# leijue222/Intra-and-Inter-Human-Relation-Network-for-MPEE

Hardware: AMD Instinct MI355X
Metric: images/sec (256x192 crops) I2R-Net HRNet-W48 inference (higher is better)
Workload: dtype f32; 1 GPU; vanilla I2R-Net HRNet-W48-S 256x192, 6 encoder layers, fp32, random weights (BASELINE configs[1]: w48_pure_en6); images_per_gpu=8, persons_per_image=4, crops_per_gpu_step=32, parallelism=single GPU, programs_per_forward=3

## Files before the change

intra-and-inter-human-relation-network-for-mpee_amd/csrc/i2r_conv.h:

```cpp
#pragma once
#include "i2r_common.h"

#ifdef I2R_TUNING
#define I2R_DBG(p) ((p).dbg)
#else
#define I2R_DBG(p) 0
#endif

namespace {

struct ConvK {
    const float* in;
    const float* in2;
    const float* w;
    const float* bias;
    const float* res1;
    const float* res2;
    const float* res_post;
    float* out;
    int n_img, in_h, in_w, in_cs, cin;
    int conv_h, conv_w, out_h, out_w, out_cs, cout, cout_pad;
    int stride, iy0, ix0, ntaps;
    int tap_kh, tap_kw;
    int out_step, out_off_y, out_off_x, rep, relu;
    int tile_h, tile_w, tiles_y, tiles_x, n_cblk;
    int ph, pw, plane;
    int ck;
    int wn;
    int dtype;
    int in16, out16;
    int dbg;
    unsigned m_cblk, m_tx, m_ty, m_pw, m_tw;
    unsigned in_bytes, w_bytes, out_bytes;
    int wn_log, npass;
    int algo, w_fwlog, w_pitch, w_half, w_nfrag, w_rcp;
    int w_seq;
    int w_band;
    unsigned w_m_cblk, w_m_img, w_m_tx;
    const float* f_t1;
    const float* f_t2;
    float* f_y;
    int f_sh1, f_sh2;
    unsigned f_bytes1, f_bytes2;
};

__device__ __forceinline__ int div_m(int n, int d, unsigned m) { return d == 1 ? n : (int)__umulhi((unsigned)n, m); }

typedef unsigned u32x4 __attribute__((ext_vector_type(4)));
typedef unsigned u32x2 __attribute__((ext_vector_type(2)));
constexpr unsigned kOOB = 0x80000000u;
__device__ __forceinline__ __amdgpu_buffer_rsrc_t make_rsrc(const void* base, unsigned bytes) {
    return __builtin_amdgcn_make_buffer_rsrc(const_cast<void*>(base), 0, base ? bytes : 0, 0x00020000);
}
__device__ __forceinline__ f32x4 buf_ld16(const __amdgpu_buffer_rsrc_t& rs, unsigned voff, int soff) {
    return __builtin_bit_cast(f32x4, __builtin_amdgcn_raw_buffer_load_b128(rs, voff, soff, 0));
}
__device__ __forceinline__ void buf_st16(const __amdgpu_buffer_rsrc_t& rs, unsigned voff, int soff, f32x4 v) {
    __builtin_amdgcn_raw_buffer_store_b128(__builtin_bit_cast(u32x4, v), rs, voff, soff, 0);
    asm volatile("s_nop 1" ::"v"(v));
}

constexpr int kMaxPP = 5;

constexpr int kMaxGroups = 4;
struct ConvGroupK {
    ConvK g[kMaxGroups];
    int blk_end[kMaxGroups];
    int n;
    const int* blk_map;
};

template <int DT>
__device__ __forceinline__ f32x4 ld_act4(const float* base, size_t off, bool h16) {
    if constexpr (DT != 0) {
        if (h16) {
            const uint2 u = *reinterpret_cast<const uint2*>(reinterpret_cast<const unsigned short*>(base) + off);
            if constexpr (DT == 1)
                return (f32x4){__uint_as_float(u.x << 16), __uint_as_float(u.x & 0xFFFF0000u), __uint_as_float(u.y << 16), __uint_as_float(u.y & 0xFFFF0000u)};
            else {
                typedef _Float16 h4 __attribute__((ext_vector_type(4)));
                const h4 h = __builtin_bit_cast(h4, u);
                return (f32x4){(float)h[0], (float)h[1], (float)h[2], (float)h[3]};
            }
        }
    }
    return *reinterpret_cast<const f32x4*>(base + off);
}
template <int DT>
__device__ __forceinline__ void st_act4(float* base, size_t off, f32x4 v, bool h16) {
    if constexpr (DT != 0) {
        if (h16) {
            uint2 u;
            if constexpr (DT == 1) {
                typedef __bf16 b4 __attribute__((ext_vector_type(4)));
                const b4 b = {(__bf16)v[0], (__bf16)v[1], (__bf16)v[2], (__bf16)v[3]};
                u = __builtin_bit_cast(uint2, b);
            } else {
                typedef _Float16 h4 __attribute__((ext_vector_type(4)));
                const h4 h = {(_Float16)v[0], (_Float16)v[1], (_Float16)v[2], (_Float16)v[3]};
                u = __builtin_bit_cast(uint2, h);
            }
            *reinterpret_cast<uint2*>(reinterpret_cast<unsigned short*>(base) + off) = u;
            return;
        }
    }
    *reinterpret_cast<f32x4*>(base + off) = v;
}

template <int DT>
__device__ __forceinline__ f32x4 buf_ld_act4(const __amdgpu_buffer_rsrc_t& rs, unsigned voff, bool h16) {
    if constexpr (DT != 0) {
        if (h16) {
            const u32x2 u = __builtin_amdgcn_raw_buffer_load_b64(rs, voff, 0, 0);
            if constexpr (DT == 1)
                return (f32x4){__uint_as_float(u.x << 16), __uint_as_float(u.x & 0xFFFF0000u), __uint_as_float(u.y << 16), __uint_as_float(u.y & 0xFFFF0000u)};
            else {
                typedef _Float16 h4 __attribute__((ext_vector_type(4)));
                const h4 h = __builtin_bit_cast(h4, u);
                return (f32x4){(float)h[0], (float)h[1], (float)h[2], (float)h[3]};
            }
        }
    }
    return buf_ld16(rs, voff, 0);
}
template <int DT>
__device__ __forceinline__ void buf_st_act4(const __amdgpu_buffer_rsrc_t& rs, unsigned voff, f32x4 v, bool h16) {
    if constexpr (DT != 0) {
        if (h16) {
            u32x2 u;
            if constexpr (DT == 1) {
                typedef __bf16 b4 __attribute__((ext_vector_type(4)));
                const b4 b = {(__bf16)v[0], (__bf16)v[1], (__bf16)v[2], (__bf16)v[3]};
                u = __builtin_bit_cast(u32x2, b);
            } else {
                typedef _Float16 h4 __attribute__((ext_vector_type(4)));
                const h4 h = {(_Float16)v[0], (_Float16)v[1], (_Float16)v[2], (_Float16)v[3]};
                u = __builtin_bit_cast(u32x2, h);
            }
            __builtin_amdgcn_raw_buffer_store_b64(u, rs, voff, 0, 0);
            return;
        }
    }
    __builtin_amdgcn_raw_buffer_store_b128(__builtin_bit_cast(u32x4, v), rs, voff, 0, 0);
}

template <int MT, int NT, int DT>
__device__ __forceinline__ void conv_epilogue(const ConvK& p, f32x4 (&acc)[MT][NT], int img, int oy0, int ox0, int wm, int n_base,
                                              int li, int g, int tile_px) {
    if ((I2R_DBG(p) & 1) && acc[0][0][0] != 12345.678f) return;
    const int j4 = li & 3;
    const int pj = li >> 2, pq = li & 3;
    const int perm_src = (g * 16 + pq * 4 + pj) * 4;
    auto to_pixel_major = [&](f32x4 v) {
        v = quad_transpose(v, j4);
#pragma unroll
        for (int e = 0; e < 4; ++e) {
            const float x = v[e];
            v[e] = __int_as_float(__builtin_amdgcn_ds_bpermute(perm_src, __float_as_int(x)));
        }
        return v;
    };
    const bool h16 = DT != 0 && p.out16;
    const unsigned esz = h16 ? 2u : 4u;
    const __amdgpu_buffer_rsrc_t rs_out = make_rsrc(p.out, p.out_bytes), rs_r1 = make_rsrc(p.res1, p.out_bytes),
                                 rs_r2 = make_rsrc(p.res2, p.out_bytes), rs_rp = make_rsrc(p.res_post, p.out_bytes);
    auto finish = [&](f32x4 t, int n, bool full, unsigned voff) {
        if (p.relu == 1) {
            t[0] = fmaxf(t[0], 0.f); t[1] = fmaxf(t[1], 0.f); t[2] = fmaxf(t[2], 0.f); t[3] = fmaxf(t[3], 0.f);
        } else if (p.relu == 2) {
#pragma unroll
            for (int e = 0; e < 4; ++e) t[e] = 0.5f * t[e] * (1.f + erff(t[e] * 0.70710678118654752f));
        }
        if (p.res_post) t += buf_ld_act4<DT>(rs_rp, voff, h16);
        if (!full) {
#pragma unroll
            for (int e = 0; e < 4; ++e)
                if (n + e >= p.cout) t[e] = 0.f;
        }
        return t;
    };
    f32x4 bias[NT];
    unsigned noff[NT];
    const bool tail = n_base + NT * 16 > p.cout || n_base + NT * 16 > p.out_cs;
#pragma unroll
    for (int nt = 0; nt < NT; ++nt) {
        const int n = n_base + nt * 16 + pq * 4;
        const bool nok = n < p.cout_pad && (n + 4 <= p.cout || n + 4 <= p.out_cs);
        noff[nt] = nok ? (unsigned)n * esz : kOOB;
        bias[nt] = n < p.cout_pad ? *reinterpret_cast<const f32x4*>(p.bias + n) : (f32x4){0.f, 0.f, 0.f, 0.f};
    }
    if (p.rep == 1 && !(I2R_DBG(p) & 16)) {
        unsigned off[MT];
#pragma unroll
        for (int mt = 0; mt < MT; ++mt) {
            const int m = (wm * MT + mt) * 16 + g * 4 + pj;
            const int ty = div_m(m, p.tile_w, p.m_tw), tx = m - ty * p.tile_w;
            const int oy = oy0 + ty, ox = ox0 + tx;
            const bool pv = m < tile_px && oy < p.conv_h && ox < p.conv_w;
            off[mt] = pv ? (unsigned)(((img * p.out_h + oy * p.out_step + p.out_off_y) * p.out_w + ox * p.out_step + p.out_off_x) * p.out_cs) * esz : kOOB;
        }
        auto at = [&](int mt, int nt) { return (tail && noff[nt] == kOOB) ? kOOB : off[mt] + noff[nt]; };
        f32x4 r[MT][NT];
#pragma unroll
        for (int mt = 0; mt < MT; ++mt)
#pragma unroll
            for (int nt = 0; nt < NT; ++nt) {
                r[mt][nt] = bias[nt];
                if (p.res1) r[mt][nt] += buf_ld_act4<DT>(rs_r1, at(mt, nt), h16);
                if (p.res2) r[mt][nt] += buf_ld_act4<DT>(rs_r2, at(mt, nt), h16);
            }
#pragma unroll
        for (int mt = 0; mt < MT; ++mt)
#pragma unroll
            for (int nt = 0; nt < NT; ++nt) {
// ... 42 lines not shown
```

intra-and-inter-human-relation-network-for-mpee_amd/csrc/i2r_conv.hip:

```cpp
#include <stdlib.h>

#include <algorithm>

#include "i2r_conv.h"

namespace {

template <int MT, int NT, int CAP, int PF>
__device__ __forceinline__ void conv_body(const ConvK& p, int bid, f32x4* lds) {
    const int tid = threadIdx.x;
    unsigned long long ts0 = 0, ts1 = 0, ts2 = 0;
    const bool stamp = (I2R_DBG(p) & 8) != 0;
    const int bid_stamp = bid;
    if (stamp) ts0 = __builtin_amdgcn_s_memtime();
    const int lane = tid & 63, wave = tid >> 6;
    const int WN = p.wn;
    const int wm = wave >> p.wn_log, wn = wave & (WN - 1);
    const int li = lane & 15, g = lane >> 4;

    int q = div_m(bid, p.n_cblk, p.m_cblk);
    const int cb = bid - q * p.n_cblk;
    bid = q;
    q = div_m(bid, p.tiles_x, p.m_tx);
    const int tile_x = bid - q * p.tiles_x;
// ... 134 lines not shown
        }
    } else {
        for (int c0 = 0; c0 < p.cin; c0 += p.ck) {
            const int ckc = min(p.ck, p.cin - c0);
            const int ncg = ckc >> 2;
            if (c0 != 0) __syncthreads();
            for (int cg0 = 0; cg0 < ncg; cg0 += 4) {
                f32x4 v[4][kMaxPP];
#pragma unroll
                for (int u = 0; u < 4; ++u)
#pragma unroll
                    for (int j = 0; j < kMaxPP; ++j)
                        v[u][j] = (j < npp && !(I2R_DBG(p) & 2)) ? buf_ld16(rs_in, goff[j] + u * 16u, (c0 + cg0 * 4) * 4) : (f32x4){0.f, 0.f, 0.f, 0.f};
                if (p.in2) {
#pragma unroll
                    for (int u = 0; u < 4; ++u)
#pragma unroll
                        for (int j = 0; j < kMaxPP; ++j)
                            if (j < npp) v[u][j] += buf_ld16(rs_in2, goff[j] + u * 16u, (c0 + cg0 * 4) * 4);
                }
#pragma unroll
                for (int u = 0; u < 4; ++u)
#pragma unroll
                    for (int j = 0; j < kMaxPP; ++j) {
                        const int pp = tid + j * 256;
                        if (j < npp && pp < phw)
                            lds[(cg0 + u) * p.plane + pp] = v[u][j];
                    }
            }
            __syncthreads();
            run_chunk(lds, c0, ckc, []() {});
        }
    }

    if (stamp) {
        ts2 = __builtin_amdgcn_s_memtime();
        ConvK q = p;
        q.res2 = nullptr;
        conv_epilogue<MT, NT, 0>(q, acc, img, oy0, ox0, wm, n_base, li, g, tile_px);
        asm volatile("s_waitcnt vmcnt(0)" ::: "memory");
        const unsigned long long ts3 = __builtin_amdgcn_s_memtime();
        if (tid == 0) {
            unsigned long long* o = reinterpret_cast<unsigned long long*>(const_cast<float*>(p.res2)) + (size_t)bid_stamp * 4;
            o[0] = ts0; o[1] = ts1; o[2] = ts2; o[3] = ts3;
            if (I2R_DBG(p) & 32) {
                const unsigned hw = __builtin_amdgcn_s_getreg((4 << 0) | (0 << 6) | (31 << 11));
                const unsigned xcc = __builtin_amdgcn_s_getreg((20 << 0) | (0 << 6) | (3 << 11));
                o[1] = ((unsigned long long)xcc << 32) | hw;
            }
        }
        return;
    }
    conv_epilogue<MT, NT, 0>(p, acc, img, oy0, ox0, wm, n_base, li, g, tile_px);
}

template <int MT, int NT, int CAP, int PF>
__global__ __launch_bounds__(256) void conv_igemm_f32(const ConvGroupK grp) {
    extern __shared__ __attribute__((aligned(16))) f32x4 lds[];
    int bid = blockIdx.x, gi = 0, start = 0;
    if (grp.blk_map) {
        const int v = __builtin_amdgcn_readfirstlane(grp.blk_map[bid]);
        gi = v >> 24;
        bid = v & 0xFFFFFF;
    } else {
#pragma unroll
        for (int i = 0; i < kMaxGroups - 1; ++i)
            if (i + 1 < grp.n && bid >= grp.blk_end[i]) { gi = i + 1; start = grp.blk_end[i]; }
    }
    conv_body<MT, NT, CAP, PF>(grp.g[gi], bid - start, lds);
}

template <int NT, int CAP, int PF>
conv_fn pick_mt(int mt) {
    switch (mt) {
        case 1: return conv_igemm_f32<1, NT, CAP, PF>;
        case 2: return conv_igemm_f32<2, NT, CAP, PF>;
        case 3: return conv_igemm_f32<3, NT, CAP, PF>;
        case 4: return conv_igemm_f32<4, NT, CAP, PF>;
    }
    return nullptr;
}

template <int CAP, int PF>
conv_fn pick_nt(int nt, int mt) {
    switch (nt) {
        case 3: return pick_mt<3, CAP, PF>(mt);
        case 4: return pick_mt<4, CAP, PF>(mt);
        case 5: return pick_mt<5, CAP, PF>(mt);
    }
    return nullptr;
}

conv_fn pick_kernel(int nt, int mt, int cap, int pf) {
    if (pf == 0) return pick_nt<4, 0>(nt, mt);
    if (pf == 1 && cap == 4) return pick_nt<4, 1>(nt, mt);
    if (pf == 1 && cap == 12) return pick_nt<12, 1>(nt, mt);
    if (pf == 2 && cap == 4) return pick_nt<4, 2>(nt, mt);
    return nullptr;
}

inline int cdiv(int a, int b) { return (a + b - 1) / b; }

}

static void copy_desc(const i2r_conv_desc* d, ConvK& k) {
    k.in = d->in; k.in2 = d->in2; k.w = d->w; k.bias = d->bias; k.res1 = d->res1; k.res2 = d->res2; k.res_post = d->res_post; k.out = d->out;
    k.n_img = d->n_img; k.in_h = d->in_h; k.in_w = d->in_w; k.in_cs = d->in_cs; k.cin = d->cin;
    k.conv_h = d->conv_h; k.conv_w = d->conv_w; k.out_h = d->out_h; k.out_w = d->out_w; k.out_cs = d->out_cs;
    k.cout = d->cout; k.cout_pad = d->cout_pad; k.stride = d->stride; k.iy0 = d->iy0; k.ix0 = d->ix0;
    k.ntaps = d->ntaps;
    k.out_step = d->out_step; k.out_off_y = d->out_off_y; k.out_off_x = d->out_off_x; k.rep = d->rep; k.relu = d->relu;
    k.dtype = d->dtype;
    k.in16 = d->in_f16; k.out16 = d->out_f16;
    k.algo = d->algo; k.w_fwlog = k.w_pitch = k.w_half = k.w_nfrag = k.w_rcp = k.w_band = 0; k.w_seq = 1;
    k.w_m_cblk = k.w_m_img = k.w_m_tx = 0; k.in_bytes = k.w_bytes = k.out_bytes = 0;
    k.m_cblk = k.m_tx = k.m_ty = k.m_pw = k.m_tw = 0; k.wn_log = 0; k.npass = 0;
    k.dbg = 0;
    k.f_t1 = d->t1; k.f_t2 = d->t2; k.f_y = d->y; k.f_sh1 = d->t1_shift; k.f_sh2 = d->t2 ? d->t2_shift : 0; k.f_bytes1 = k.f_bytes2 = 0;
}

constexpr int kWinoMaxSeq = 8;
constexpr int kWinoRunPasses = 6;
constexpr int kWinoMinWg = 512;
static long long wino_runs(const ConvK& k, int mt) { return (((long long)k.w_nfrag + mt - 1) / mt + k.w_seq - 1) / k.w_seq; }

static int prepare_wino(const i2r_conv_desc* d, int force_mt, ConvK& k, int* nt_out, int* mt_out, int* cap_out, int* pf_out, size_t* lds_out,
                        long long* nblk_out) {
    I2R_CHECK_ARG(d->dtype == 0 && !d->in_f16 && !d->out_f16, "i2r_conv: the Winograd kernels are fp32");
    I2R_CHECK_ARG(d->stride == 1 && d->ntaps == 9 && d->iy0 == -1 && d->ix0 == -1 && d->rep == 1 && d->out_step == 1 && d->out_off_y == 0 &&
                      d->out_off_x == 0 && d->in2 == nullptr,
                  "i2r_conv: algo 1 (Winograd) needs a plain 3x3 stride-1 pad-1 convolution");
    for (int t = 0; t < 9; ++t) I2R_CHECK_ARG(d->dy[t] == t / 3 && d->dx[t] == t % 3, "i2r_conv: algo 1 needs row-major 3x3 taps");
    I2R_CHECK_ARG(d->relu == 0 || d->relu == 1, "i2r_conv: algo 1 has no GELU epilogue");
    I2R_CHECK_ARG((long long)d->n_img * d->in_h * d->in_w * d->in_cs < (1ll << 29) && (long long)d->n_img * d->out_h * d->out_w * d->out_cs < (1ll << 29) &&
                      (long long)16 * d->cin * d->cout_pad < (1ll << 29),
                  "i2r_conv: algo 1 addresses its tensors through buffer descriptors of < 2 GiB");
    I2R_CHECK_ARG(d->conv_h == d->in_h && d->conv_w == d->in_w && d->out_h == d->conv_h && d->out_w == d->conv_w, "i2r_conv: algo 1 geometry");
    if (d->t1) {
        I2R_CHECK_ARG(d->y != nullptr, "i2r_conv: a fused input (t1) needs y");
        I2R_CHECK_ARG(d->in_cs == d->cin, "i2r_conv: fused input: y is complete only when the conv reads every channel (cin=%d in_cs=%d)", d->cin, d->in_cs);
        for (int t = 0; t < (d->t2 ? 2 : 1); ++t) {
            const int sh = t ? d->t2_shift : d->t1_shift;
            I2R_CHECK_ARG((sh == 1 || sh == 2) && d->in_h % (1 << sh) == 0 && d->in_w % (1 << sh) == 0,
                          "i2r_conv: fused input: t%d_shift %d must be 1 or 2 and the %dx%d map divisible by the scale", t + 1, sh, d->in_h, d->in_w);
        }
        const void* others[] = {d->in, d->t1, d->t2, d->out, d->res1, d->res2, d->res_post};
        for (const void* o : others) I2R_CHECK_ARG((const void*)d->y != o, "i2r_conv: fused input: y aliases another tensor of the launch");
        I2R_CHECK_ARG(d->t1 != (const float*)d->out && d->t2 != (const float*)d->out, "i2r_conv: out aliases a fused-input term");
    }
    const int nfrag = d->cout_pad / 16;
    const int nt = nfrag % 3 == 0 ? 3 : (nfrag % 4 == 0 ? 4 : 0);
    I2R_CHECK_ARG(nt != 0, "i2r_conv: algo 1 needs cout_pad=%d to be a multiple of 48 or 64", d->cout_pad);
    const int mt = force_mt ? force_mt : (d->mt ? d->mt : 1);
    I2R_CHECK_ARG(mt == 1, "i2r_conv: algo 1 takes mt 1 (got %d)", mt);
    I2R_CHECK_ARG(d->seq >= 0 && d->seq <= kWinoMaxSeq, "i2r_conv: algo 1 runs 1..%d fragments per workgroup (seq=%d; 0 = choose)", kWinoMaxSeq, d->seq);
    int fw = 0;
    if (d->tile_w) {
        I2R_CHECK_ARG(d->tile_w == 16 || d->tile_w == 8 || d->tile_w == 4, "i2r_conv: algo 1 fragment width %d (16, 8, 4)", d->tile_w);
        fw = d->tile_w / 2;
    } else {
        long long best = -1;
        for (int cand : {8, 4, 2}) {
            const long long n = (long long)cdiv(d->conv_w, 2 * cand) * cdiv(d->conv_h, 32 / cand);
            if (best < 0 || n < best) { best = n; fw = cand; }
        }
    }
    copy_desc(d, k);
    k.w_fwlog = fw == 8 ? 3 : (fw == 4 ? 2 : 1);
    k.tile_w = 2 * fw; k.tile_h = 32 / fw;
    k.tiles_x = cdiv(d->conv_w, k.tile_w); k.tiles_y = cdiv(d->conv_h, k.tile_h);
    k.n_cblk = nfrag / nt;
    k.ph = k.tile_h + 2; k.pw = k.tile_w + 2;
    k.w_half = fw + 1;
    k.w_pitch = fw == 8 ? 20 : (fw == 4 ? 10 : 9);
    k.plane = cdiv(k.ph * k.w_pitch, 16) * 16;
    k.w_rcp = (65536 + k.pw - 1) / k.pw;
    k.in_bytes = (unsigned)((long long)d->n_img * d->in_h * d->in_w * d->in_cs * 4);
    k.w_bytes = (unsigned)((long long)16 * d->cin * d->cout_pad * 4);
    k.out_bytes = (unsigned)((long long)d->n_img * d->out_h * d->out_w * d->out_cs * 4);
    if (d->t1) k.f_bytes1 = (unsigned)((long long)d->n_img * (d->in_h >> d->t1_shift) * (d->in_w >> d->t1_shift) * d->in_cs * 4);
    if (d->t2) k.f_bytes2 = (unsigned)((long long)d->n_img * (d->in_h >> d->t2_shift) * (d->in_w >> d->t2_shift) * d->in_cs * 4);
    auto magic = [](int d) { return d == 1 ? 0u : (unsigned)(((1ull << 32) + d - 1) / d); };
    k.w_m_cblk = magic(k.n_cblk); k.w_m_img = magic(k.tiles_y * k.tiles_x); k.w_m_tx = magic(k.tiles_x);
    k.tap_kw = k.tap_kh = 3;
    k.ck = 16; k.wn = 1;
    const long long nf = (long long)d->n_img * k.tiles_y * k.tiles_x;
    I2R_CHECK_ARG(nf > 0 && nf * k.n_cblk < (1ll << 20) && k.tiles_y * k.tiles_x < 2048 && k.n_cblk < 2048, "i2r_conv: algo 1 grid (%lld fragments)", nf);
    k.w_nfrag = (int)nf;
    k.w_seq = d->seq ? d->seq : 1;
#ifdef I2R_TUNING
    {
        static const int dbg = getenv("I2R_CONV_DBG") ? atoi(getenv("I2R_CONV_DBG")) : 0;
        k.dbg = dbg;
    }
#endif
    *nt_out = nt; *mt_out = mt; *cap_out = 0; *pf_out = 100;
    *lds_out = i2r_conv_wino_lds(nt, mt, k.plane);
    *nblk_out = wino_runs(k, mt) * k.n_cblk;
    return I2R_OK;
}

static void wino_choose_seq(ConvK* g, const i2r_conv_desc* const* descs, int n, int mt) {
    auto total = [&]() { long long t = 0; for (int i = 0; i < n; ++i) t += wino_runs(g[i], mt) * g[i].n_cblk; return t; };
    long long at_one = 0;
    for (int i = 0; i < n; ++i) at_one += ((long long)g[i].w_nfrag + mt - 1) / mt * g[i].n_cblk;
    const long long floor_wg = std::min<long long>(at_one, kWinoMinWg);
    for (int i = 0; i < n; ++i)
        if (descs[i]->seq == 0) g[i].w_seq = std::max(1, std::min(kWinoMaxSeq, kWinoRunPasses / (g[i].cin >> 4)));
    while (total() < floor_wg) {
        int pick = -1;
        for (int i = 0; i < n; ++i) {
            if (descs[i]->seq != 0 || g[i].w_seq == 1) continue;
            const int len = g[i].w_seq * (g[i].cin >> 4);
            if (pick < 0 || len > g[pick].w_seq * (g[pick].cin >> 4) || (len == g[pick].w_seq * (g[pick].cin >> 4) && g[i].cin > g[pick].cin)) pick = i;
        }
        if (pick < 0) break;
        --g[pick].w_seq;
    }
}

static int prepare(const i2r_conv_desc* d, int force_mt, int force_cap, int force_pf, ConvK& k, int* nt_out, int* mt_out, int* cap_out,
                   int* pf_out, size_t* lds_out, long long* nblk_out) {
    I2R_CHECK_ARG(d && d->in && d->w && d->bias && d->out, "i2r_conv: null pointer");
    I2R_CHECK_ARG(d->cin > 0 && d->cin % 16 == 0 && d->cin <= d->in_cs && d->in_cs % 4 == 0,
                  "i2r_conv: cin=%d must be a multiple of 16 and <= in_cs=%d (in_cs %% 4 == 0)", d->cin, d->in_cs);
    I2R_CHECK_ARG(d->cout > 0 && d->cout_pad % 16 == 0 && d->cout <= d->cout_pad && d->cout <= d->out_cs && d->out_cs % 4 == 0,
                  "i2r_conv: cout=%d cout_pad=%d out_cs=%d", d->cout, d->cout_pad, d->out_cs);
    I2R_CHECK_ARG(d->stride == 1 || d->stride == 2, "i2r_conv: stride %d", d->stride);
    I2R_CHECK_ARG(d->dtype >= 0 && d->dtype <= 2 && (d->dtype == 0 || d->in2 == nullptr), "i2r_conv: dtype %d", d->dtype);
    I2R_CHECK_ARG((d->in_f16 == 0 || d->in_f16 == 1) && (d->out_f16 == 0 || d->out_f16 == 1) && (d->dtype != 0 || (!d->in_f16 && !d->out_f16)),
                  "i2r_conv: 16-bit activation storage (in_f16=%d out_f16=%d) needs a 16-bit operand type (dtype=%d)", d->in_f16, d->out_f16, d->dtype);
    I2R_CHECK_ARG(!d->in_f16 || d->in_cs % 8 == 0, "i2r_conv: 16-bit input needs in_cs %% 8 == 0 (in_cs=%d)", d->in_cs);
    I2R_CHECK_ARG(d->ntaps >= 1 && d->ntaps <= I2R_MAX_TAPS, "i2r_conv: ntaps %d", d->ntaps);
    I2R_CHECK_ARG(d->rep >= 1 && d->out_step >= 1, "i2r_conv: rep/out_step");
    I2R_CHECK_ARG((d->conv_h - 1) * d->out_step + d->out_off_y + d->rep <= d->out_h &&
                      (d->conv_w - 1) * d->out_step + d->out_off_x + d->rep <= d->out_w,
                  "i2r_conv: destination grid exceeds out tensor");
    I2R_CHECK_ARG(d->in2 != (const float*)d->out && d->in != (const float*)d->out, "i2r_conv: out aliases in");
    I2R_CHECK_ARG(d->algo == 0 || d->algo == 1, "i2r_conv: algo %d", d->algo);
    I2R_CHECK_ARG(d->t1 ? d->algo == 1 : (!d->t2 && !d->y), "i2r_conv: a fused input (t1, t2, y) needs algo 1 and starts with t1");
    if (d->algo == 1) return prepare_wino(d, force_mt, k, nt_out, mt_out, cap_out, pf_out, lds_out, nblk_out);

    int max_dy = 0, max_dx = 0;
    for (int t = 0; t < d->ntaps; ++t) {
        I2R_CHECK_ARG(d->dy[t] >= 0 && d->dx[t] >= 0, "i2r_conv: negative tap offset");
        if (d->dy[t] > max_dy) max_dy = d->dy[t];
        if (d->dx[t] > max_dx) max_dx = d->dx[t];
    }

    const int nfrag = d->cout_pad / 16;
    int nt = 0;
    for (int cand : {3, 4, 5})
        if (nfrag % cand == 0) { nt = cand; break; }
    I2R_CHECK_ARG(nt != 0, "i2r_conv: cout_pad=%d is not a multiple of 48, 64 or 80", d->cout_pad);
    int wn = d->wn;
    if (wn == 0) {
        const int nb = nfrag / nt;
        wn = (nb % 4 == 0) ? 4 : (nb % 2 == 0) ? 2 : 1;
        if (wn == 4 && d->cout_pad < 192) wn = 2;
    }
    I2R_CHECK_ARG((wn == 1 || wn == 2 || wn == 4) && (nfrag / nt) % wn == 0, "i2r_conv: wn=%d does not divide cout", wn);
    const int wm = 4 / wn;

    int th = d->tile_h, tw = d->tile_w, mt = force_mt ? force_mt : d->mt;
    if (th == 0 || tw == 0) {
        tw = d->conv_w <= 16 ? d->conv_w : (d->conv_w % 16 == 0 ? 16 : (d->conv_w % 12 == 0 ? 12 : 8));
        if (mt == 0) mt = 2;
        th = (wm * mt * 16) / tw;
        if (th < 1) th = 1;
        if (th > d->conv_h) th = d->conv_h;
    }
    if (mt == 0) mt = cdiv(th * tw, wm * 16);
    I2R_CHECK_ARG(mt >= 1 && mt <= 4 && th * tw <= wm * mt * 16, "i2r_conv: tile %dx%d does not fit wm=%d mt=%d", th, tw, wm, mt);

    copy_desc(d, k);
    k.tile_h = th; k.tile_w = tw;
    k.tiles_y = cdiv(d->conv_h, th); k.tiles_x = cdiv(d->conv_w, tw);
    k.n_cblk = nfrag / (nt * wn);
    k.ph = (th - 1) * d->stride + max_dy + 1;
    k.pw = (tw - 1) * d->stride + max_dx + 1;
    I2R_CHECK_ARG(k.ph * k.pw <= kMaxPP * 256, "i2r_conv: patch %dx%d too large", k.ph, k.pw);
#ifdef I2R_TUNING
    static const int plane_pad = getenv("I2R_CONV_PLANE_PAD") ? atoi(getenv("I2R_CONV_PLANE_PAD")) : 0;
#else
    constexpr int plane_pad = 0;
#endif
    k.plane = cdiv(k.ph * k.pw, 16) * 16 + plane_pad;
    k.tap_kw = max_dx + 1;
    k.tap_kh = max_dy + 1;
    for (int t = 0; t < d->ntaps; ++t)
        I2R_CHECK_ARG(d->dy[t] == t / k.tap_kw && d->dx[t] == t % k.tap_kw && d->ntaps == (max_dy + 1) * (max_dx + 1),
                      "i2r_conv: taps must form a dense row-major kh x kw grid");
    const int npp = cdiv(k.ph * k.pw, 256);
#ifdef I2R_TUNING
    static const int pf_env = getenv("I2R_CONV_PF") ? atoi(getenv("I2R_CONV_PF")) : 1;
#else
    constexpr int pf_env = 1;
#endif
    const int cin_g = d->dtype == 0 ? d->cin / 4 : (d->cin / 8 + 3) / 4 * 4;
    const int g_ch = d->dtype == 0 ? 4 : 8;
    int pf = (pf_env && d->ck == 0 && npp <= 2 && cin_g % 4 == 0) ? npp : 0;
    int cap = 4;
    if (force_pf >= 0) {
        I2R_CHECK_ARG(force_pf == 0 || (npp <= force_pf && d->ck == 0 && cin_g % 4 == 0), "i2r_conv: grouped members disagree on the staging mode");
        pf = force_pf;
    }
    int ck = d->ck;
    size_t lds_bytes;
    if (pf > 0) {
        int ckg = 4;
#ifdef I2R_TUNING
        static const int cap_env = getenv("I2R_CONV_CAP") ? atoi(getenv("I2R_CONV_CAP")) : 12;
#else
        constexpr int cap_env = 12;
#endif
        const int cap_max = std::min(cap_env, d->dtype == 0 ? 12 : 8);
        const int cap_lim = force_pf >= 0 ? force_cap : (pf == 1 ? cap_max : 4);
        for (int cand : {12, 8, 4})
            if (cand <= cap_lim && cin_g % cand == 0 && (size_t)2 * cand * k.plane * 16 <= 40 * 1024) { ckg = cand; break; }
        cap = force_pf >= 0 ? force_cap : (ckg > 4 ? cap_max : 4);
        ck = ckg * g_ch;
        lds_bytes = (size_t)2 * ckg * k.plane * 16;
    } else if (d->dtype != 0) {
        const int g8_pad = (d->cin / 8 + 3) / 4 * 4;
        int fit = (24 * 1024 / (k.plane * 16)) / 4 * 4;
        if (fit < 4) fit = 4;
        const int nchunk = cdiv(g8_pad, fit);
        const int ckg = cdiv(cdiv(g8_pad, nchunk), 4) * 4;
        ck = ckg * 8;
        lds_bytes = (size_t)ckg * k.plane * 16;
    } else {
        if (ck == 0) {
            const int budget = 20 * 1024;
            int fit = (budget / (k.plane * 16)) * 4;
            fit = fit < 16 ? 16 : fit / 16 * 16;
            const int nchunk = cdiv(d->cin, fit);
            ck = cdiv(cdiv(d->cin, nchunk), 16) * 16;
        }
        I2R_CHECK_ARG(ck % 16 == 0 && ck >= 16, "i2r_conv: ck=%d", ck);
        lds_bytes = (size_t)(ck / 4) * k.plane * 16;
    }
    k.ck = ck;
    I2R_CHECK_ARG(lds_bytes <= 160 * 1024, "i2r_conv: LDS %zu B", lds_bytes);
    k.wn = wn;
    {
        const long long esz_in = d->in_f16 ? 2 : 4, esz_out = d->out_f16 ? 2 : 4;
        const long long inb = (long long)d->n_img * d->in_h * d->in_w * d->in_cs * esz_in, outb = (long long)d->n_img * d->out_h * d->out_w * d->out_cs * esz_out;
        const long long wb = d->dtype == 0 ? (long long)d->ntaps * d->cin * d->cout_pad * 4 : (long long)d->ntaps * ((d->cin / 8 + 3) / 4 * 4) * 8 * d->cout_pad * 2;
        I2R_CHECK_ARG(inb < (1ll << 31) && outb < (1ll << 31) && wb < (1ll << 31), "i2r_conv: tensors of 2 GiB and more are not supported (in %lld, out %lld, weights %lld bytes)", inb, outb, wb);
        k.in_bytes = (unsigned)inb; k.out_bytes = (unsigned)outb; k.w_bytes = (unsigned)wb;
        auto magic = [](int d) { return d == 1 ? 0u : (unsigned)(((1ull << 32) + d - 1) / d); };
        k.m_cblk = magic(k.n_cblk); k.m_tx = magic(k.tiles_x); k.m_ty = magic(k.tiles_y); k.m_pw = magic(k.pw); k.m_tw = magic(k.tile_w);
        k.wn_log = wn == 4 ? 2 : (wn == 2 ? 1 : 0);
        k.npass = d->dtype == 0 ? d->cin / ck : ((d->cin / 8 + 3) / 4 * 4) / (ck / 8);
    }
// ... 136 lines not shown
```

intra-and-inter-human-relation-network-for-mpee_amd/csrc/i2r_conv_wino.hip:

```cpp
#include "i2r_conv.h"

namespace {

constexpr int kWinoPatchMax = 108;

typedef const ConvK __attribute__((address_space(4)))* ConvKArg;

template <int MT, int NT, bool FIN>
__device__ __forceinline__ void conv_wino_body(const ConvGroupK& grp, ConvKArg args) {
    extern __shared__ __attribute__((aligned(16))) f32x4 lds[];
    const int tid = threadIdx.x, lane = tid & 63;
    const int wi = __builtin_amdgcn_readfirstlane(tid >> 6);
    const int li = lane & 15, g = lane >> 4;

    int bid = blockIdx.x, gi = 0;
    if (grp.blk_map) {
        const int v = __builtin_amdgcn_readfirstlane(grp.blk_map[bid]);
        gi = v >> 24;
        bid = v & 0xFFFFFF;
    } else {
        int start = 0;
#pragma unroll
        for (int i = 0; i < kMaxGroups - 1; ++i)
            if (i + 1 < grp.n && bid >= grp.blk_end[i]) { gi = i + 1; start = grp.blk_end[i]; }
        bid -= start;
    }
    const ConvK& p = grp.g[gi];
    const bool stamp = (I2R_DBG(p) & 8) != 0;
    unsigned long long ts0 = 0, ts1 = 0, ts2 = 0;
    if (stamp) ts0 = __builtin_amdgcn_s_memtime();

    int wg, cb;
    if (grp.blk_map) {
        wg = div_m(bid, p.n_cblk, p.w_m_cblk);
        cb = bid - wg * p.n_cblk;
    } else {
        const int q = bid >> 3, qq = div_m(q, p.n_cblk, p.w_m_cblk);
        cb = q - qq * p.n_cblk;
        wg = (bid & 7) * p.w_band + qq;
    }
    const int run0 = wg * p.w_seq;
    const int nrun = min(p.w_seq, (p.w_nfrag + MT - 1) / MT - run0);
    if (nrun <= 0) return;
    const int fwl = p.w_fwlog, FW = 1 << fwl;
    const int pitch = p.w_pitch, half = p.w_half, plane = p.plane;
    const int n_base = cb * NT * 16;

    constexpr int NIT = (MT * kWinoPatchMax * 4 + 255) / 256;
    const __amdgpu_buffer_rsrc_t rs_in = __builtin_amdgcn_make_buffer_rsrc(const_cast<float*>(p.in), 0, p.in_bytes, 0x00020000);
    const __amdgpu_buffer_rsrc_t rs_w = __builtin_amdgcn_make_buffer_rsrc(const_cast<float*>(p.w), 0, p.w_bytes, 0x00020000);
    unsigned goff[NIT];
    int lslot[NIT];
    constexpr int kOwn = 1 << 30;
    const bool fin = FIN && p.f_t1 != nullptr, fin2 = fin && p.f_t2 != nullptr;
    const __amdgpu_buffer_rsrc_t rs_t1 = make_rsrc(fin ? p.f_t1 : nullptr, p.f_bytes1), rs_t2 = make_rsrc(fin2 ? p.f_t2 : nullptr, p.f_bytes2),
                                 rs_y = make_rsrc(fin ? p.f_y : nullptr, p.in_bytes);
    unsigned goff1[FIN ? NIT : 1], goff2[FIN ? NIT : 1];
    const int cg = tid & 3;
    auto patch_pixel = [&](const auto& pq, int t, int k, int& f, int& row, int& col) {
        const int PC = pq.pw, PP = pq.ph * pq.pw;
        const int pix = (t + k * 256) >> 2;
        int pp = pix;
        f = 0;
#pragma unroll
        for (int m = 1; m <= MT; ++m)
            if (pix >= m * PP) { f = m; pp = pix - m * PP; }
        row = (pp * pq.w_rcp) >> 16;
        col = pp - row * PC;
    };
#pragma unroll
    for (int k = 0; k < NIT; ++k) {
        int f, row, col;
        patch_pixel(p, tid, k, f, row, col);
        lslot[k] = f < MT ? (f * 4 + cg) * plane + row * pitch + (col & 1) * half + (col >> 1) : -1;
        if constexpr (FIN) {
            if (f < MT && row >= 1 && row < p.ph - 1 && col >= 1 && col < p.pw - 1) lslot[k] |= kOwn;
        }
    }
    auto lane_now = []() {
        int l;
        asm volatile("v_mbcnt_lo_u32_b32 %0, -1, 0\n\tv_mbcnt_hi_u32_b32 %0, -1, %0" : "=v"(l));
        return l;
    };
    int f_img[MT], f_oy[MT], f_ox[MT];
    bool f_ok[MT];
    auto set_fragment = [&](int fg, int t, const auto& ps) {
#pragma unroll
        for (int mt = 0; mt < MT; ++mt) {
            int fid = fg * MT + mt;
            f_ok[mt] = fid < ps.w_nfrag;
            if (!f_ok[mt]) fid = 0;
            f_img[mt] = div_m(fid, (ps.tiles_y * ps.tiles_x), ps.w_m_img);
            const int rem = fid - f_img[mt] * (ps.tiles_y * ps.tiles_x);
            const int fy = div_m(rem, ps.tiles_x, ps.w_m_tx);
            f_oy[mt] = fy * (32 >> fwl);
            f_ox[mt] = (rem - fy * ps.tiles_x) * (2 * FW);
        }
#pragma unroll
        for (int k = 0; k < NIT; ++k) {
            int f, row, col;
            patch_pixel(ps, t, k, f, row, col);
            int img = f_img[0], oy = f_oy[0], ox = f_ox[0];
            bool ok = f_ok[0] && f < MT;
#pragma unroll
            for (int m = 1; m < MT; ++m)
                if (f == m) { img = f_img[m]; oy = f_oy[m]; ox = f_ox[m]; ok = f_ok[m]; }
            const int iy = oy - 1 + row, ix = ox - 1 + col;
            const bool in_img = ok && (unsigned)iy < (unsigned)ps.in_h && (unsigned)ix < (unsigned)ps.in_w;
            goff[k] = in_img ? (unsigned)(((img * ps.in_h + iy) * ps.in_w + ix) * ps.in_cs + (t & 3) * 4) * 4u : kOOB;
            if constexpr (FIN) {
                const int s1 = ps.f_sh1, s2 = ps.f_sh2;
                goff1[k] = in_img ? (unsigned)(((img * (ps.in_h >> s1) + (iy >> s1)) * (ps.in_w >> s1) + (ix >> s1)) * ps.in_cs + (t & 3) * 4) * 4u : kOOB;
                goff2[k] = in_img ? (unsigned)(((img * (ps.in_h >> s2) + (iy >> s2)) * (ps.in_w >> s2) + (ix >> s2)) * ps.in_cs + (t & 3) * 4) * 4u : kOOB;
            }
        }
    };
    f32x4 v[NIT];
    auto stage_load = [&](int c0) {
#pragma unroll
        for (int k = 0; k < NIT; ++k)
            v[k] = (I2R_DBG(p) & 2) ? (f32x4){0.f, 0.f, 0.f, 0.f}
                                    : __builtin_bit_cast(f32x4, __builtin_amdgcn_raw_buffer_load_b128(rs_in, goff[k], c0 * 4, 0));
    };
    f32x4 vt[FIN ? NIT : 1];
    auto stage_load_t1 = [&](int c0) {
        if constexpr (FIN) {
            if (fin) {
#pragma unroll
                for (int k = 0; k < NIT; ++k) vt[k] = buf_ld16(rs_t1, goff1[k], c0 * 4);
            }
        }
    };
    auto stage_mid = [&](int c0) {
        if constexpr (FIN) {
            if (fin2) {
#pragma unroll
                for (int k = 0; k < NIT; ++k) {
                    v[k] += vt[k];
                    vt[k] = buf_ld16(rs_t2, goff2[k], c0 * 4);
                }
            }
        }
    };
    auto stage_store = [&](f32x4* buf, int c0) {
        if constexpr (FIN) {
            if (fin) {
#pragma unroll
                for (int k = 0; k < NIT; ++k) {
                    v[k] += vt[k];
                    v[k][0] = fmaxf(v[k][0], 0.f); v[k][1] = fmaxf(v[k][1], 0.f); v[k][2] = fmaxf(v[k][2], 0.f); v[k][3] = fmaxf(v[k][3], 0.f);
                    if (cb == 0) buf_st16(rs_y, (unsigned)lslot[k] >= (unsigned)kOwn ? goff[k] : kOOB, c0 * 4, v[k]);
                }
            }
// ... 38 lines not shown
#pragma unroll
        for (int nt = 0; nt < NT; ++nt)
            b[nt] = __builtin_bit_cast(f32x4, __builtin_amdgcn_raw_buffer_load_b128(rs_w, wlane + nt * 256u, (I2R_DBG(p) & 4) ? 0 : wp, 0));
    };

    f32x4 acc[4][MT][NT];
    const int npass = p.cin >> 4;
    const int bufsz = MT * 4 * plane;
    f32x4 a[MT][4], b0[NT], b1[NT];
#define WINO_MMA(J, B, FIRST)                                                                                   \
    if (!(I2R_DBG(p) & 16))                                                                                     \
    _Pragma("unroll") for (int s = 0; s < 4; ++s) _Pragma("unroll") for (int mt = 0; mt < MT; ++mt)             \
        _Pragma("unroll") for (int nt = 0; nt < NT; ++nt)                                                       \
            acc[J][mt][nt] = mfma16(a[mt][J][s], B[nt][s], ((FIRST) && s == 0) ? (f32x4){0.f, 0.f, 0.f, 0.f} : acc[J][mt][nt]);
#define WINO_PASS(PASS, FIRST)                                                                   \
    {                                                                                            \
        const int pass_ = (PASS);                                                                \
        f32x4* cur = lds + (pass_ & 1) * bufsz;                                                  \
        f32x4* nxt = lds + ((pass_ + 1) & 1) * bufsz;                                            \
        const bool more = pass_ + 1 < npass;                                                     \
        if (more) { stage_load((pass_ + 1) * 16); stage_load_t1((pass_ + 1) * 16); }             \
        load_a(cur, a);                                                                          \
        wp += inc_j; fetch_b(b1);                                                                \
        WINO_MMA(0, b0, FIRST)                                                                   \
        wp += inc_j; fetch_b(b0);                                                                \
        WINO_MMA(1, b1, FIRST)                                                                   \
        if (more) stage_mid((pass_ + 1) * 16);                                                   \
        wp += inc_j; fetch_b(b1);                                                                \
        WINO_MMA(2, b0, FIRST)                                                                   \
        if (more) { wp += inc_wrap; fetch_b(b0); }                                               \
        WINO_MMA(3, b1, FIRST)                                                                   \
        if (more) stage_store(nxt, (pass_ + 1) * 16);                                            \
        if (!(I2R_DBG(p) & 64)) __syncthreads();                                                 \
    }
    float* const Tl = reinterpret_cast<float*>(lds);
    constexpr int TW = NT * 16;
    constexpr int TPL = MT * 16 * TW;
    const bool tail = n_base + NT * 16 > p.cout || n_base + NT * 16 > p.out_cs;

    for (int fs = 0; fs < nrun; ++fs) {
    {
        const int tid_s = wi * 64 + lane_now();
        ConvKArg ps_ = args + gi;
        asm volatile("" : "+s"(ps_));
        set_fragment(run0 + fs, tid_s, *ps_);
        abase_f = abase;
        asm volatile("" : "+v"(abase_f));
#pragma unroll
        for (int k = 0; k < NIT; ++k) asm volatile("" : "+v"(lslot[k]));
    }
    wp = wp0;
    stage_load(0);
    stage_load_t1(0);
    if constexpr (FIN) {
        if (fin2) {
            f32x4 vu[NIT];
#pragma unroll
            for (int k = 0; k < NIT; ++k) vu[k] = buf_ld16(rs_t2, goff2[k], 0);
#pragma unroll
            for (int k = 0; k < NIT; ++k) {
                v[k] += vt[k];
                vt[k] = vu[k];
            }
        }
    }
    fetch_b(b0);
    if (fs) __syncthreads();
    stage_store(lds, 0);
    __syncthreads();
    if (stamp) ts1 = __builtin_amdgcn_s_memtime();
    WINO_PASS(0, true)
    for (int pass = 1; pass < npass; ++pass) WINO_PASS(pass, false)
    if (stamp) ts2 = __builtin_amdgcn_s_memtime();

    const int tid_f = wi * 64 + lane_now();
    ConvKArg pe_ = args + gi;
    asm volatile("" : "+s"(pe_));
    const auto& pe = *pe_;
    const float* const res2e = stamp ? nullptr : pe.res2;
    const unsigned out_bytes = pe.out_bytes;
    const __amdgpu_buffer_rsrc_t rs_out = make_rsrc(pe.out, out_bytes), rs_r1 = make_rsrc(pe.res1, out_bytes), rs_r2 = make_rsrc(res2e, out_bytes),
                                 rs_rp = make_rsrc(pe.res_post, out_bytes);
#pragma unroll
    for (int mt = 0; mt < MT; ++mt)
#pragma unroll
        for (int nt = 0; nt < NT; ++nt) {
            const f32x4 t0 = acc[0][mt][nt] + acc[1][mt][nt] + acc[2][mt][nt];
            const f32x4 t1 = acc[1][mt][nt] - acc[2][mt][nt] - acc[3][mt][nt];
            float* q = Tl + (wi * 2) * TPL + (mt * 16 + ((tid_f & 63) >> 4) * 4) * TW + nt * 16 + (tid_f & 15);
#pragma unroll
            for (int r = 0; r < 4; ++r) {
                q[r * TW] = t0[r];
                q[TPL + r * TW] = t1[r];
            }
        }
    unsigned obase[MT];
    const int q4 = tid_f & 3, px = tid_f >> 2;
    const bool hi = (px & 2) != 0;
    const int n0 = n_base + q4 * 4;
    f32x4 r[MT][NT];
#pragma unroll
    for (int mt = 0; mt < MT; ++mt) {
        const int t = px >> 2;
        const int oy = f_oy[mt] + 2 * (t >> fwl) + (hi ? 1 : 0);
        const int ox = f_ox[mt] + 2 * (t & (FW - 1)) + (px & 1);
        const bool ok = f_ok[mt] && oy < pe.conv_h && ox < pe.conv_w;
        obase[mt] = ok ? (unsigned)(((f_img[mt] * pe.out_h + oy) * pe.out_w + ox) * pe.out_cs + n0) * 4u : kOOB;
#pragma unroll
        for (int k = 0; k < NT; ++k) {
            r[mt][k] = *reinterpret_cast<const f32x4*>(pe.bias + n0 + 16 * k);
            if (!(I2R_DBG(p) & 1)) {
                if (pe.res1) r[mt][k] += buf_ld16(rs_r1, obase[mt] + 64u * k, 0);
                if (res2e) r[mt][k] += buf_ld16(rs_r2, obase[mt] + 64u * k, 0);
            }
        }
    }
    const float* const tq = Tl + ((px & 1) + (hi ? 2 : 0)) * TPL + (px >> 2) * TW + q4 * 4;
    const float sgn = hi ? -1.f : 1.f;
    __syncthreads();
#pragma unroll
    for (int mt = 0; mt < MT; ++mt)
#pragma unroll
        for (int k = 0; k < NT; ++k) {
            const float* q = tq + mt * 16 * TW + 16 * k;
            const f32x4 u0 = *reinterpret_cast<const f32x4*>(q);
            const f32x4 u1 = *reinterpret_cast<const f32x4*>(q + 2 * TPL);
            const f32x4 u2 = *reinterpret_cast<const f32x4*>(q + 4 * TPL);
            f32x4 y = u0 + sgn * (u1 + u2) + r[mt][k];
            if (pe.relu) { y[0] = fmaxf(y[0], 0.f); y[1] = fmaxf(y[1], 0.f); y[2] = fmaxf(y[2], 0.f); y[3] = fmaxf(y[3], 0.f); }
            unsigned off = obase[mt] + 64u * k;
            if (pe.res_post) y += buf_ld16(rs_rp, off, 0);
            if (tail) {
                const int n = n0 + 16 * k;
                if (!(n + 4 <= pe.cout || n + 4 <= pe.out_cs)) off = kOOB;
#pragma unroll
                for (int e = 0; e < 4; ++e)
                    if (n + e >= pe.cout) y[e] = 0.f;
            }
            if (!(I2R_DBG(p) & 1) || y[0] == 12345.678f) __builtin_amdgcn_raw_buffer_store_b128(__builtin_bit_cast(u32x4, y), rs_out, off, 0, 0);
        }
    }
#undef WINO_PASS
#undef WINO_MMA
    if (stamp) {
        asm volatile("s_waitcnt vmcnt(0)" ::: "memory");
        const unsigned long long ts3 = __builtin_amdgcn_s_memtime();
        if (tid == 0) {
            unsigned long long* o = reinterpret_cast<unsigned long long*>(const_cast<float*>(p.res2)) + (size_t)bid * 4;
            o[0] = ts0; o[1] = ts1; o[2] = ts2; o[3] = ts3;
        }
    }
}

__device__ __forceinline__ ConvKArg wino_args() {
    static_assert(offsetof(ConvGroupK, g) == 0, "the members lead the kernel argument");
    return (ConvKArg)__builtin_amdgcn_kernarg_segment_ptr();
}

template <int MT, int NT>
__global__ __launch_bounds__(256, (MT == 1 ? (NT == 3 ? 4 : 3) : 2)) void conv_wino_f32(const ConvGroupK grp) {
    conv_wino_body<MT, NT, false>(grp, wino_args());
}

template <int MT, int NT>
__global__ __launch_bounds__(256, (MT == 1 ? (NT == 3 ? 4 : 3) : 2)) void conv_wino_fin_f32(const ConvGroupK grp) {
    conv_wino_body<MT, NT, true>(grp, wino_args());
}

}

void* i2r_pick_conv_wino(int nt, int mt, int fin) {
    conv_fn fn = nullptr;
    if (mt == 1 && nt == 3) fn = fin ? conv_wino_fin_f32<1, 3> : conv_wino_f32<1, 3>;
    if (mt == 1 && nt == 4) fn = fin ? conv_wino_fin_f32<1, 4> : conv_wino_f32<1, 4>;
    return reinterpret_cast<void*>(fn);
}

size_t i2r_conv_wino_lds(int nt, int mt, int plane) {
    const size_t stage = (size_t)2 * mt * 4 * plane * 16;
    const size_t xchg = (size_t)4 * 2 * mt * 16 * nt * 16 * 4;
    return stage > xchg ? stage : xchg;
}
```

intra-and-inter-human-relation-network-for-mpee_amd/engine.py:

```python
import ctypes as C
import math
import os

import torch

from . import cabi
from .pack import (PRECISIONS, PackedConv, Packer, _m16, _r16, fold_bn, pack_frag, pack_frag32, pack_k4, pack_k8,
                   winograd_weights)


def wino_fragment(conv_h, conv_w):
    best = None
    for fw in (8, 4, 2):
        n = -(-conv_w // (2 * fw)) * -(-conv_h // (32 // fw))
        if best is None or n < best[0]:
            best = (n, 2 * fw, 32 // fw)
    return best[1], best[2]


LP1X1 = True
LP1X1_MAX_PIX = 65536
_HRT_FUSED_ATTN = (78, 156, 312)
_HRT_FUSED_MLP = (78, 156, 312)
_MLP_VARIANT = {78: 1, 156: 2, 312: 2}
PAIR1X1 = True
FUSE_IN = True
PRUNE_FUSE = True
WINOGRAD = True
WINO_SEQ = True
PROFILER_ATTACHED = bool(os.environ.get("ROCP_TOOL_LIBRARIES") or os.environ.get("ROCPROFILER_LIBRARY_CTOR") or os.environ.get("HSA_TOOLS_LIB")
                         or any(t in os.environ.get("LD_PRELOAD", "") for t in ("rocprof", "roctracer", "rocprofiler")))
DEVICE_SYNC = not PROFILER_ATTACHED


class Act:
    __slots__ = ("t", "n", "h", "w", "c", "cs", "dt")
    TORCH_DT = {0: torch.float32, 1: torch.bfloat16, 2: torch.float16}

    def __init__(self, t, n, h, w, c, cs, dt=0):
        self.t, self.n, self.h, self.w, self.c, self.cs, self.dt = t, n, h, w, c, cs, dt

    def view(self):
        return self.t.view(self.TORCH_DT[self.dt])[:self.n * self.h * self.w * self.cs].view(self.n, self.h, self.w, self.cs)

    @property
    def ptr(self):
        return self.t.data_ptr()


class _RawAct:
    __slots__ = ("ptr", "n", "h", "w", "c", "cs", "dt")

    def __init__(self, ptr, like, n=None):
        self.ptr, self.n, self.h, self.w, self.c, self.cs, self.dt = ptr, like.n if n is None else n, like.h, like.w, like.c, like.cs, 0


_MT_EFF = {1: 0.62, 2: 0.9, 3: 1.0, 4: 0.9}


def choose_tile(conv_h, conv_w, wm, stride, max_d, n_img, n_cblk, force_mt=0, want_cost=False):
    best = None
    cands_w = sorted({w for w in (conv_w, 48, 32, 24, 16, 12, 8, 6, 4) if w <= conv_w and w <= 48})
    for mt in ((force_mt,) if force_mt else (1, 2, 3, 4)):
        cap = wm * mt * 16
        for tw in cands_w:
            th = min(conv_h, cap // tw)
            if th < 1:
                continue
            ph, pw = (th - 1) * stride + max_d + 1, (tw - 1) * stride + max_d + 1
            if ph * pw > 1280:
                continue
            tiles = -(-conv_h // th) * -(-conv_w // tw)
            blocks = tiles * n_img * n_cblk
            rounds = -(-blocks // 256)
            halo = ph * pw / float(th * stride * tw * stride)
            cost = rounds * (cap / _MT_EFF[mt]) * (1.0 + 0.08 * (halo - 1.0))
            if best is None or cost < best[0] - 1e-9:
                best = (cost, th, tw, mt)
    assert best is not None, "no tile for %dx%d" % (conv_h, conv_w)
    if want_cost:
        return best
    return best[1], best[2], best[3]


_LPT_CACHE = {}
_LPT_DEV = {}


def lpt_block_table(device, counts, works):
    key = (str(device), tuple(counts), tuple(works))
    t = _LPT_DEV.get(key)
    if t is None:
        ck = (tuple(counts), tuple(works), 256)
        if ck not in _LPT_CACHE:
            _LPT_CACHE[ck] = lpt_block_order(counts, works)
        t = _LPT_DEV[key] = torch.tensor(_LPT_CACHE[ck], dtype=torch.int32, device=device)
    return t


def lpt_block_order(counts, works, n_cu=256):
    import heapq
    items = sorted(((w, g, i) for g, (c, w) in enumerate(zip(counts, works)) for i in range(c)),
                   key=lambda t: (-t[0], t[1], t[2]))
    heap = [(0, b) for b in range(n_cu)]
    bins = [[] for _ in range(n_cu)]
    for w, g, i in items:
        load, b = heapq.heappop(heap)
        bins[b].append((g << 24) | i)
        heapq.heappush(heap, (load + w, b))
    out, r = [], 0
    while len(out) < len(items):
        for b in range(n_cu):
            if r < len(bins[b]):
                out.append(bins[b][r])
        r += 1
    return out


def conv_split(cout_pad):
    nfrag = cout_pad // 16
    nt = next(c for c in (3, 4, 5) if nfrag % c == 0)
    nb = nfrag // nt
    wn = 4 if nb % 4 == 0 else 2 if nb % 2 == 0 else 1
    return nt, wn


class Program:
    def __init__(self, device):
        self.device = device
        self.ops = []
        self.keep = []
        self.pool = {}
        self.pending = []
        self.lane_pool = {}
        self.lane_ctx = 0
        self.groupings = []
        self.enc_stacks = []
        self.split_counters = []
        self.captures = []
        self.query = None
        self.store_dt = 0
        self.in_fork = False
        self.nbytes = 0
        self._snap = None
        self._next_slot = -1
        self._c_ops = None
        self._flags_op = None
        self.uses_lanes = False
        self.device_sync = False
        self._flags = None
        self._events = None
        self._tev = None
        self._capture_ws = None

    def alloc(self, n, h, w, c, dt=0):
        cs = _r16(c)
        numel = (n * h * w * cs + 1) // 2 if dt else n * h * w * cs
        lst = (self.lane_pool.get((self.lane_ctx, numel)) if self.in_fork else None) or self.pool.get(numel)
        if lst:
            t = lst.pop()
        else:
            t = torch.empty(numel, dtype=torch.float32, device=self.device)
            self.nbytes += numel * 4
            self.keep.append(t)
        return Act(t, n, h, w, c, cs, dt)

    def release(self, *acts):
        for a in acts:
            if a is None:
                continue
            if self.in_fork:
                self.lane_pool.setdefault((self.lane_ctx, a.t.numel()), []).append(a.t)
            else:
                self.pool.setdefault(a.t.numel(), []).append(a.t)

    def release_deferred(self, *acts):
        for a in acts:
            if self.in_fork:
                self.pending.append(a.t)
            else:
                self.pool.setdefault(a.t.numel(), []).append(a.t)

    def stem(self, st, n, h, w, in_ptr=0, lane=0, n_src=None, out_dt=0):
        out = self.alloc(n, (h - 1) // 2 + 1, (w - 1) // 2 + 1, st["cout"], out_dt)
        self.keep.append(st)
        ns = n if n_src is None else n_src
        a = cabi.StemArgs(in_ptr, st["w"].data_ptr(), st["bias"].data_ptr(), out.ptr, n, st["cin"], h, w, st["cout"], out.cs, ns, ns, out_dt)
        self.ops.append((cabi.OP_STEM, lane, a))
        return out, a

    def pe_res_stem(self, st, n, h, w, lane=0, n_src=None):
        out = self.alloc(n, (h - 1) // 2 + 1, (w - 1) // 2 + 1, st["cout"])
        self.keep.append(st)
        ns = n if n_src is None else n_src
        a = cabi.PeResArgs(0, st["w_pre"].data_ptr(), st["w7"].data_ptr(), st["bias"].data_ptr(), out.ptr, n, h, w, st["cout"], out.cs, ns, ns)
        self.ops.append((cabi.OP_PE_RES_STEM, lane, a))
        return out, a

    def conv(self, x, pc, relu=False, res1=None, res2=None, res_post=None, in2=None, up=1, out=None, out_step=1,
             out_off=(0, 0), out_hw=None, lane=0, group=None, act=None, out_dt=None, fuse_in=None):
        assert x.cs >= pc.cin_pad and x.c == pc.cin, "conv input channels %d/%d vs weight %d" % (x.c, x.cs, pc.cin)
        assert x.dt in (0, pc.dtype), "16-bit stored input needs the matching 16-bit conv (input %d, conv %d)" % (x.dt, pc.dtype)
        if (LP1X1 and pc.w_lp1 is not None and fuse_in is None and group is None and in2 is None and up == 1 and out_step == 1 and tuple(out_off) == (0, 0)
                and out_hw is None and x.n * x.h * x.w <= LP1X1_MAX_PIX and (out is None or (out.n, out.h, out.w) == (x.n, x.h, x.w))
                and (out is None or out.cs >= pc.cout_pad) and all(r is None or out is None or r.cs == out.cs for r in (res1, res2, res_post))
                and all(r is None or r.cs >= pc.cout_pad for r in (res1, res2, res_post))):
            return self.conv1x1_lp(x, pc, relu=relu, res1=res1, res2=res2, res_post=res_post, out=out, lane=lane, act=act, out_dt=out_dt)
        k = pc.ksize
        if pc.stride == 1:
            conv_h, conv_w = x.h, x.w
        else:
            conv_h, conv_w = (x.h - 1) // 2 + 1, (x.w - 1) // 2 + 1
        if up > 1:
            out_step = up
        if out is None:
            oh, ow = out_hw if out_hw else (conv_h * out_step, conv_w * out_step)
            out = self.alloc(x.n, oh, ow, pc.cout, x.dt if out_dt is None else out_dt)
        assert out.cs >= pc.cout_pad or out.cs >= pc.cout
        assert out.dt in (0, pc.dtype) and all(r is None or r.dt == out.dt for r in (res1, res2, res_post)), "residuals share the output's storage type"
        self._check_like(out, res1, res2, res_post)
        if in2 is not None and (in2.n, in2.h, in2.w, in2.cs) != (x.n, x.h, x.w, x.cs):
            raise ValueError("conv second input is [%d, %d, %d, cs %d], the first [%d, %d, %d, cs %d]" % (in2.n, in2.h, in2.w, in2.cs, x.n, x.h, x.w, x.cs))
        self.keep.append(pc)
        d = cabi.ConvDesc()
        d.in_, d.in2, d.w, d.bias = x.ptr, (in2.ptr if in2 is not None else None), pc.w.data_ptr(), pc.bias.data_ptr()
        d.res1 = res1.ptr if res1 is not None else None
        d.res2 = res2.ptr if res2 is not None else None
        d.res_post = res_post.ptr if res_post is not None else None
        d.out = out.ptr
        d.n_img, d.in_h, d.in_w, d.in_cs, d.cin = x.n, x.h, x.w, x.cs, pc.cin_pad
        d.conv_h, d.conv_w, d.out_h, d.out_w, d.out_cs = conv_h, conv_w, out.h, out.w, out.cs
        d.cout, d.cout_pad, d.stride, d.iy0, d.ix0 = pc.cout, pc.cout_pad, pc.stride, pc.iy0, pc.ix0
        d.ntaps = len(pc.taps)
        for i, (dy, dx) in enumerate(pc.taps):
            d.dy[i], d.dx[i] = dy, dx
        d.out_step, d.out_off_y, d.out_off_x, d.rep = out_step, out_off[0], out_off[1], up
        d.relu = int(relu) if act is None else act
        d.dtype = pc.dtype
        d.in_f16, d.out_f16 = int(x.dt != 0), int(out.dt != 0)
        wino = (WINOGRAD and pc.w_wino is not None and pc.dtype == 0 and in2 is None and up == 1 and out_step == 1 and tuple(out_off) == (0, 0)
                and (out.h, out.w) == (conv_h, conv_w) and d.relu in (0, 1))
        if fuse_in is not None:
            terms, y = fuse_in
            if not (wino and self.fuse_in_ok(x, terms, pc)):
                raise ValueError("fuse_in needs an fp32 Winograd conv over every channel of x and 1 or 2 terms at 1/2 or 1/4 of its map")
            assert all(t.cs == x.cs and t.dt == 0 and t.n == x.n for t in terms) and (y.n, y.h, y.w, y.cs, y.dt) == (x.n, x.h, x.w, x.cs, 0)
            sh = [{2: 1, 4: 2}[x.h // t.h] for t in terms]
            assert all((t.h << k, t.w << k) == (x.h, x.w) for t, k in zip(terms, sh))
            d.t1, d.t1_shift, d.y = terms[0].ptr, sh[0], y.ptr
            if len(terms) > 1:
                d.t2, d.t2_shift = terms[1].ptr, sh[1]
        if wino:
            nfrag = pc.cout_pad // 16
            nt = 3 if nfrag % 3 == 0 else 4
            fw, fh = wino_fragment(conv_h, conv_w)
            d.algo, d.w = 1, pc.w_wino.data_ptr()
            mt = 1
            d.tile_h, d.tile_w, d.mt, d.wn, d.ck = fh, fw, mt, 1, 0
            d.seq = 0 if WINO_SEQ else 1
            n_frag = x.n * -(-conv_h // fh) * -(-conv_w // fw)
            geo = ("wino", -(-n_frag // mt) * (nfrag // nt))
            key = ("wino", nt, mt)
        else:
            nt, wn = conv_split(pc.cout_pad)
            n_cblk = (pc.cout_pad // 16) // (nt * wn)
            max_d = max(max(t) for t in pc.taps)
            th, tw, mt = choose_tile(conv_h, conv_w, 4 // wn, pc.stride, max_d, x.n, n_cblk, force_mt=1 if pc.stride == 2 else 0)
            d.tile_h, d.tile_w, d.mt, d.wn, d.ck = th, tw, mt, wn, 0
            geo = (conv_h, conv_w, 4 // wn, pc.stride, max_d, x.n, n_cblk)
            key = nt
        if group is not None:
            group.append((d, geo, key))
        elif wino:
            self.flush_group([(d, geo, key)], lane=lane)
        else:
            self.ops.append((cabi.OP_CONV, lane, d))
        return out

    @staticmethod
    def fuse_in_ok(x, terms, pc):
        return (WINOGRAD and pc.w_wino is not None and pc.dtype == 0 and x.dt == 0 and x.c == pc.cin and x.cs == pc.cin_pad
                and 1 <= len(terms) <= 2 and all((t.h * 2, t.w * 2) == (x.h, x.w) or (t.h * 4, t.w * 4) == (x.h, x.w) for t in terms))

    @staticmethod
    def _group_tiles(group):
        best = None
        s2 = all(geo[3] == 2 for _, geo, _ in group)
        for mt in ((1,) if s2 else (2, 3, 4, 1)):
            try:
                tiles = [choose_tile(*geo, force_mt=mt, want_cost=True) for _, geo, _ in group]
            except AssertionError:
                continue
            blocks = 0
            work = 0.0
            for (d, geo, _), t in zip(group, tiles):
                conv_h, conv_w, wm, stride, max_d, n_img, n_cblk = geo
                nb = -(-conv_h // t[1]) * -(-conv_w // t[2]) * n_img * n_cblk
                blocks += nb
                work += nb * (wm * mt * 16 / _MT_EFF[mt]) * d.cin * d.ntaps
            cost = work * max(1.0, 256.0 / blocks)
            if best is None or cost < best[0]:
                best = (cost, mt, tiles)
        _, mt, tiles = best
        return mt, tiles

    def flush_group(self, group, lane=0):
        if not group:
            return
        nts = {g[2] for g in group}
        wino = group[0][0].algo == 1
        if (len(group) == 1 and not wino) or len(nts) != 1 or len(group) > cabi.MAX_GROUP:
            for m in list(group):
                if m[0].algo == 1:
                    self.flush_group([m], lane=lane)
                else:
                    self.ops.append((cabi.OP_CONV, lane, m[0]))
            del group[:]
            return
        if not wino:
            mt, tiles = self._group_tiles(group)
        order = sorted(range(len(group)), key=lambda i: -(group[i][0].cin * group[i][0].ntaps))
        a = cabi.ConvGroupArgs()
        counts, works = [], []
        for slot, i in enumerate(order):
            d, geo, _ = group[i]
            a.d[slot] = C.pointer(d)
            self.keep.append(d)
            if wino:
                counts.append(geo[1])
            else:
                d.tile_h, d.tile_w, d.mt = tiles[i][1], tiles[i][2], mt
                conv_h, conv_w, wm, stride, max_d, n_img, n_cblk = geo
                counts.append(-(-conv_h // d.tile_h) * -(-conv_w // d.tile_w) * n_img * n_cblk)
            works.append(d.cin * d.ntaps)
        a.n = len(group)
        if not wino and len(set(works)) > 1:
            bm = lpt_block_table(self.device, counts, works)
            self.keep.append(bm)
            a.block_map, a.map_len = bm.data_ptr(), bm.numel()
        self.ops.append((cabi.OP_CONV_GROUP, lane, a))
        del group[:]

    def channel_slice(self, a, c0, c):
        assert c0 % 16 == 0 and c0 + c <= a.cs
        words = c0 // 2 if a.dt else c0
        return Act(a.t[words:], a.n, a.h, a.w, c, a.cs, a.dt)

    def stem_conv2_layer1(self, a, conv2, blocks):
        first = blocks[0]
        assert "c3ds" in first, "layer1.0 carries the downsample"
        cx, cm = conv2.cout, first["c2"].cout
        cat = self.alloc(a.n, (a.h - 1) // 2 + 1, (a.w - 1) // 2 + 1, cx + cm, a.dt)
        x, t2 = self.channel_slice(cat, 0, cx), self.channel_slice(cat, cx, cm)
        self.conv(a, conv2, relu=True, out=x)
        self.release(a)
        t1 = self.conv(x, first["c1"], relu=True)
        self.conv(t1, first["c2"], relu=True, out=t2)
        def pair_ok(pa, pb):
            return (pa.w_frag is not None and pa.cin in (64, 128) and pa.cout % 32 == 0 and pa.cout == pa.cout_pad
                    and (pb is None or (pb.w_frag is not None and pb.cout == 64 and pb.cin == pa.cout)))
        nxt = [b["c1"] for b in blocks[1:]] + [None]
        if PAIR1X1 and a.dt == 0 and pair_ok(first["c3ds"], nxt[0]) and all(pair_ok(b["c3"], nxt[i]) for i, b in enumerate(blocks[1:], 1)):
            self.release(t1)
            y, t1 = self.conv1x1_pair(cat, first["c3ds"], None, blocks[1]["c1"] if len(blocks) > 1 else None)
            self.release(cat)
            for i, blk in enumerate(blocks[1:], 1):
                t2 = self.conv(t1, blk["c2"], relu=True)
                self.release(t1)
                yn, t1 = self.conv1x1_pair(t2, blk["c3"], y, blocks[i + 1]["c1"] if i + 1 < len(blocks) else None)
                self.release(t2, y)
                y = yn
            return y
        y = self.conv(cat, first["c3ds"], relu=True)
        self.release(t1, cat)
        x = y
        for blk in blocks[1:]:
            t1 = self.conv(x, blk["c1"], relu=True)
            t2 = self.conv(t1, blk["c2"], relu=True)
            y = self.conv(t2, blk["c3"], relu=True, res1=x)
            self.release(t1, t2, x)
            x = y
        return x

    def deconv(self, x, pcs, relu=True, res_post=None, lane=0):
        out = self.alloc(x.n, 2 * x.h, 2 * x.w, pcs[(0, 0)].cout, x.dt)
        grp = []
        for (py, px), pc in pcs.items():
            self.conv(x, pc, relu=relu, res_post=res_post, out=out, out_step=2, out_off=(py, px), lane=lane, group=grp)
        self.flush_group(grp, lane=lane)
        return out

    def rows_gather(self, src, crop_map, lane=0):
        out = self.alloc(len(crop_map), src.h, src.w, src.c)
        assert out.cs == src.cs, "rows_gather copies whole rows: source and output need the same row stride (%d vs %d)" % (src.cs, out.cs)
        m = torch.tensor(list(crop_map), dtype=torch.int32).to(self.device)
        self.keep.append(m)
        a = cabi.GatherArgs(src.ptr, out.ptr, m.data_ptr(), len(crop_map), src.h * src.w * src.cs)
        self.ops.append((cabi.OP_ROWS_GATHER, lane, a))
        return out

    def rows_gather_multi(self, segments, lane=0):
        assert 1 <= len(segments) <= cabi.MAX_GATHER_SEGS, "rows_gather_multi: %d segments (1..%d)" % (len(segments), cabi.MAX_GATHER_SEGS)
        a = cabi.GatherMultiArgs()
        a.n_seg = len(segments)
        for g, (src, out, table, n_out, n_src, src_crop, out_crop) in zip(a.seg, segments):
            row = src.h * src.w * src.cs * (2 if src.dt else 4)
            assert (out.h, out.w, out.cs, out.dt) == (src.h, src.w, src.cs, src.dt), "rows_gather_multi copies whole rows of one stride and type"
            assert row % 16 == 0 and table.dtype == torch.int32 and table.numel() >= n_out
            assert 0 <= out_crop and out_crop + n_out <= out.n and 0 <= src_crop and src_crop + n_src <= src.n
            self.keep.append(table)
            g.src, g.out, g.map = src.ptr + row * src_crop, out.ptr + row * out_crop, table.data_ptr()
            g.n_out, g.n_src, g.row_bytes = n_out, n_src, row
        self.ops.append((cabi.GROUPS_OP_ROWS_GATHER_MULTI, lane, a))
        return a

    def view_scramble(self, o, person_map, n_images, max_persons, c, lane=0):
        out = self.alloc(len(person_map), o.h, o.w, c)
        m = torch.tensor(list(person_map), dtype=torch.int32).to(self.device)
        self.keep.append(m)
        a = cabi.ScrambleArgs(o.ptr, out.ptr, m.data_ptr(), len(person_map), n_images, max_persons, c, out.cs, o.h * o.w)
        assert o.cs == out.cs and o.n == n_images * max_persons
        self.ops.append((cabi.OP_VIEW_SCRAMBLE, lane, a))
        return out

    def pe_cat_vec(self, fc, n, h, w, th, tw, out, c0, lane=0, n_src=None):
        rate = int(math.log(w // tw, 2))
        assert (out.n, out.h, out.w) == (n, th, tw) and out.dt == 0 and c0 + fc["vec"] <= out.cs
        self.keep.append(fc)
        ns = n if n_src is None else n_src
        a = cabi.PeCatVecArgs(0, fc["w"].data_ptr(), fc["b"].data_ptr(), out.ptr, n, h, w, th, tw, rate, fc["vec"], out.cs, c0, out.cs, ns, ns)
        self.ops.append((cabi.OP_PE_CAT_VEC, lane, a))
        return a

    def maxpool(self, x, lane=0, out=None):
        assert x.dt == 0, "fp32 kernel: the producer must store fp32 (conv(..., out_dt=0))"
        if out is None:
            out = self.alloc(x.n, (x.h - 1) // 2 + 1, (x.w - 1) // 2 + 1, x.c)
        assert (out.n, out.h, out.w) == (x.n, (x.h - 1) // 2 + 1, (x.w - 1) // 2 + 1) and out.cs >= x.cs and out.dt == 0
        a = cabi.PoolArgs(x.ptr, out.ptr, x.n, x.h, x.w, x.cs, x.cs, out.cs)
        self.ops.append((cabi.OP_MAXPOOL, lane, a))
        return out

    def layernorm(self, x, ln, eps=1e-6, lane=0, out_dt=0):
        assert x.dt == 0, "fp32 kernel: the producer must store fp32 (conv(..., out_dt=0))"
        out = self.alloc(x.n, x.h, x.w, x.c, out_dt)
        self.keep.append(ln)
        a = cabi.LnArgs(x.ptr, ln["w"].data_ptr(), ln["b"].data_ptr(), out.ptr, x.n * x.h * x.w, x.c, x.cs, eps, out_dt)
        self.ops.append((cabi.OP_LAYERNORM, lane, a))
        return out

    def winattn(self, qkv, bias, c, heads, lane=0):
        hs = heads * Packer.HEAD_PAD
        assert qkv.cs == 3 * hs, (qkv.cs, hs)
        out = self.alloc(qkv.n, qkv.h, qkv.w, hs)
        self.keep.append(bias)
        a = cabi.WinAttnArgs(qkv.ptr, bias.data_ptr(), out.ptr, qkv.n, qkv.h, qkv.w, c, hs, heads)
        self.ops.append((cabi.OP_WINATTN, lane, a))
        return out

    def hrt_attn(self, x, ab, eps=1e-6, lane=0, variant=None):
        assert x.dt == 0 and x.c == ab["c"] and x.cs == ab["cs"]
        if not variant or (variant == 1 and ab["c"] not in (78, 156)):
            variant = 2
        out = self.alloc(x.n, x.h, x.w, x.c)
        self.keep.append(ab)
        a = cabi.HrtAttnArgs(x.ptr, out.ptr, ab["ln"]["w"].data_ptr(), ab["ln"]["b"].data_ptr(), ab["wqkv"].data_ptr(), ab["bqkv"].data_ptr(),
                             ab["wo"].data_ptr(), ab["bo"].data_ptr(), x.n, x.h, x.w, x.c, x.cs, ab["heads"], eps, ab["dtype"], variant)
        self.ops.append((cabi.OP_HRT_ATTN, lane, a))
        return out

    def hrt_mlp(self, x, mb, eps=1e-6, lane=0, variant=None):
        assert x.dt == 0 and x.c == mb["c"] and x.cs == mb["cs"]
        if not variant or (variant == 1 and mb["c"] > 156):
            variant = _MLP_VARIANT[mb["c"]]
        out = self.alloc(x.n, x.h, x.w, x.c)
        self.keep.append(mb)
        a = cabi.HrtMlpArgs(x.ptr, out.ptr, mb["ln"]["w"].data_ptr(), mb["ln"]["b"].data_ptr(), mb["w1"].data_ptr(), mb["b1"].data_ptr(),
                            mb["wdw"].data_ptr(), mb["bdw"].data_ptr(), mb["w2"].data_ptr(), mb["b2"].data_ptr(), x.n, x.h, x.w, x.c, x.cs,
                            mb["hidden_pad"], eps, mb["dtype"], variant)
        self.ops.append((cabi.OP_HRT_MLP, lane, a))
        return out

    def dwconv(self, x, dw, stride=1, act=0, lane=0):
        assert x.dt == 0 or stride == 1
        assert x.c == dw["c"] and x.cs == dw["cs"]
        out = self.alloc(x.n, (x.h - 1) // stride + 1, (x.w - 1) // stride + 1, x.c, x.dt)
        self.keep.append(dw)
        a = cabi.DwArgs(x.ptr, dw["w"].data_ptr(), dw["bias"].data_ptr(), out.ptr, x.n, x.h, x.w, x.c, x.cs, stride, act, x.dt)
        self.ops.append((cabi.OP_DWCONV, lane, a))
        return out

    def upsample_add(self, low, res, out, act=0, lane=0):
        lows = list(low) if isinstance(low, (list, tuple)) else [low]
        assert 1 <= len(lows) <= 3
        sc = [out.h // t.h for t in lows]
        assert all(t.h * s == out.h and t.w * s == out.w and t.cs == out.cs == res.cs and t.n == out.n for t, s in zip(lows, sc))
        a = cabi.UpArgs(lows[0].ptr, res.ptr, out.ptr, lows[0].n, lows[0].h, lows[0].w, sc[0], lows[0].c, lows[0].cs, act,
                        lows[1].ptr if len(lows) > 1 else None, lows[2].ptr if len(lows) > 2 else None,
                        sc[1] if len(lows) > 1 else 1, sc[2] if len(lows) > 2 else 1)
        self.ops.append((cabi.OP_UPSAMPLE, lane, a))
        return out

    @staticmethod
    def _check_like(out, *residuals):
        for r in residuals:
            if r is not None and (r.n, r.h, r.w, r.cs) != (out.n, out.h, out.w, out.cs):
                raise ValueError("conv residual is [%d, %d, %d, row %d], the output [%d, %d, %d, row %d]" % (r.n, r.h, r.w, r.cs, out.n, out.h, out.w, out.cs))

    def conv1x1_lp(self, x, pc, relu=False, res1=None, res_post=None, out=None, lane=0, act=None, out_dt=None, res2=None):
        if out is None:
            out = self.alloc(x.n, x.h, x.w, pc.cout, x.dt if out_dt is None else out_dt)
        assert out.cs >= pc.cout_pad and out.dt in (0, pc.dtype) and all(r is None or (r.dt == out.dt and r.cs == out.cs) for r in (res1, res2, res_post))
        self._check_like(out, res1, res2, res_post)
        self.keep.append(pc)
        a = cabi.Conv1x1LpArgs(x.ptr, pc.w_lp1.data_ptr(), pc.bias.data_ptr(), res1.ptr if res1 is not None else None,
                               res_post.ptr if res_post is not None else None, out.ptr, x.n * x.h * x.w, pc.cin_pad, pc.cout_pad, x.cs, out.cs,
                               (int(relu) if act is None else act), pc.dtype, int(x.dt != 0), int(out.dt != 0), 0,
                               res2.ptr if res2 is not None else None)
        self.ops.append((cabi.OP_CONV1X1_LP, lane, a))
        return out

    def conv1x1_pair(self, x, pa, res, pb, lane=0):
        assert x.dt == 0 and pa.w_frag is not None and pa.ksize == 1 and pa.cin == x.cs and (pb is None or (pb.w_frag is not None and pb.cin == pa.cout))
        y = self.alloc(x.n, x.h, x.w, pa.cout)
        z = self.alloc(x.n, x.h, x.w, pb.cout) if pb is not None else None
        assert res is None or (res.cs == y.cs and res.dt == 0 and res.n * res.h * res.w == y.n * y.h * y.w)
        self.keep.extend([pa, pb])
        a = cabi.Conv1x1PairArgs(x.ptr, pa.w_frag.data_ptr(), pa.bias.data_ptr(), res.ptr if res is not None else None, y.ptr,
                                 pb.w_frag.data_ptr() if pb is not None else None, pb.bias.data_ptr() if pb is not None else None,
                                 z.ptr if z is not None else None, x.n * x.h * x.w, pa.cin, pa.cout, pb.cout if pb is not None else 0,
                                 x.cs, y.cs, z.cs if z is not None else 0, 1, 1, 0)
# ... 264 lines not shown

    def set_groups(self, grouping, grp_off_host):
        offs = tuple(int(o) for o in grp_off_host)
        if grouping["current"] == offs:
            return
        assert len(offs) <= grouping["goff"].numel()
        lens = [offs[i + 1] - offs[i] for i in range(len(offs) - 1)]
        assert all(l > 0 for l in lens)
        nq, nq16, nq64, nq192 = (sum(-(-l // t) for l in lens) for t in (32, 16, 64, 192))
        grouping["goff"][:len(offs)].copy_(torch.tensor(offs, dtype=torch.int32).pin_memory(), non_blocking=True)
        for d, dt in grouping["descs"]:
            d.n_grp, d.n_qtiles32, d.n_qtiles16, d.n_qtiles64 = len(offs) - 1, nq, nq16, nq64
            d.n_qtiles192 = nq192
            d.dtype = dt
        for a in grouping.get("mh", ()):
            a.n_grp, a.n_qtiles16, a.n_qtiles32, a.n_qtiles64 = len(offs) - 1, nq16, nq, nq64
        grouping["current"] = offs

    def fork(self, mask):
        if not any(k == cabi.OP_LANE_FLAGS for k, _, _ in self.ops):
            self.ops.append((cabi.OP_LANE_FLAGS, 0, None))
        self.ops.append((cabi.OP_FORK, mask, None))
        self.in_fork = True

    def _flush_lane_pools(self):
        for t in self.pending:
            self.pool.setdefault(t.numel(), []).append(t)
        self.pending = []
        for (_, numel), lst in self.lane_pool.items():
            self.pool.setdefault(numel, []).extend(lst)
        self.lane_pool = {}

    def records(self, lanes):
        assert self.in_fork and self._snap is None
        slots, region = {}, 0
        for l in lanes:
            region |= 1 << l
        for l in lanes:
            slot = self._next_slot = (self._next_slot + 1) % 8
            self.ops.append((cabi.OP_RECORD, l | slot << 8 | region << 16, None))
            slots[l] = slot
        self._snap = (self.pending, self.lane_pool)
        self.pending, self.lane_pool = [], {}
        return slots

    def wait(self, lane, slot):
        self.ops.append((cabi.OP_WAIT, lane | slot << 8, None))

    def all_waited(self):
        pend, lp = self._snap
        self._snap = None
        for t in pend:
            self.pool.setdefault(t.numel(), []).append(t)
        for (_, numel), lst in lp.items():
            self.pool.setdefault(numel, []).extend(lst)

    def join(self, mask):
        assert self._snap is None
        self.ops.append((cabi.OP_JOIN, mask, None))
        self.in_fork = False
        self._flush_lane_pools()
        self.lane_ctx = 0

    def finalize(self):
        arr = (cabi.Op * len(self.ops))()
        for i, (kind, lane, st) in enumerate(self.ops):
            arr[i].kind, arr[i].lane = kind, lane
            arr[i].args = C.cast(C.pointer(st), C.c_void_p) if st is not None else None
        self._c_ops = arr
        self._flags_op = next((i for i, (kind, _, _) in enumerate(self.ops) if kind == cabi.OP_LANE_FLAGS), None)
        self.uses_lanes = any(lane != 0 or kind in cabi.SYNC_OPS for kind, lane, _ in self.ops)

    def run(self, side_streams=None, events=None):
        L = cabi.lib()
        cur = torch.cuda.current_stream(self.device).cuda_stream
        if side_streams is None:
            streams = (C.c_void_p * 4)(cur, cur, cur, cur)
        else:
            streams = (C.c_void_p * 4)(cur, *[s.cuda_stream for s in side_streams])
        evs = None
        if self._flags_op is not None:
            spin = side_streams is not None and DEVICE_SYNC and lanes_independent(self.device, side_streams, cur)
            self._c_ops[self._flags_op].args = self._lane_flags().data_ptr() if spin else None
            self.device_sync = spin
        if self.uses_lanes:
            if events is None:
                events = self._own_events()
            evs = (C.c_void_p * len(events))(*[e.cuda_event for e in events])
        try:
            if Program.timing_log is not None:
                self._run_timed(L, streams, evs)
            else:
                cabi.check(L.i2r_run_program(self._c_ops, len(self.ops), streams, evs), "i2r_run_program")
        except Exception:
            for t in self.split_counters:
                t.zero_()
            raise

    timing_log = None
    timing_markers = True

    def _run_timed(self, L, streams, evs):
        n = len(self.ops)
        key = (tuple(streams), Program.timing_markers)
        if self._tev is None or self._tev[0] != key:
            t0, t1, seen = [None] * n, [None] * n, set()
            for i, (kind, lane, st) in enumerate(self.ops):
                if kind in cabi.SYNC_OPS:
                    continue
                t1[i] = torch.cuda.Event(enable_timing=True)
                t1[i].record()
                if Program.timing_markers or streams[lane] not in seen:
                    seen.add(streams[lane])
                    t0[i] = torch.cuda.Event(enable_timing=True)
                    t0[i].record()
            torch.cuda.synchronize(self.device)
            self._tev = (key, t0, t1, (C.c_void_p * n)(*[e.cuda_event if e is not None else None for e in t0]),
                         (C.c_void_p * n)(*[e.cuda_event if e is not None else None for e in t1]))
        _, t0, t1, a0, a1 = self._tev
        cabi.check(L.i2r_run_program_timed(self._c_ops, n, streams, evs, a0, a1), "i2r_run_program_timed")
        Program.timing_log.append((self, t0, t1, key[0]))

    def _lane_flags(self):
        if self._flags is None:
            self._flags = torch.zeros(64, dtype=torch.int32, device=self.device)
        return self._flags

    def sync_timed_out(self):
        return self._flags is not None and bool(self._flags[63].item())

    def _own_events(self):
        if self._events is None:
            self._events = [torch.cuda.Event(enable_timing=False) for _ in range(16)]
            for e in self._events:
                e.record()
        return self._events


class _PendingFuse:
    __slots__ = ("base", "terms")

    def __init__(self, base, terms):
        self.base, self.terms = base, terms


class HRNetW48:

    def __init__(self, pk, p, extra):
        self.extra = extra
        s2, s3 = extra["STAGE2"], extra["STAGE3"]
        self.stride = 4 * 2 ** (s3["NUM_BRANCHES"] - 1)
        self.stem1 = pk.stem(p + "conv1", p + "bn1")
        self.conv2 = pk.conv(p + "conv2", p + "bn2", stride=2)
        self.layer1 = pk.bottlenecks(p + "layer1", 4)
        self.t1 = [pk.conv(p + "transition1.0.0", p + "transition1.0.1"),
                   pk.conv(p + "transition1.1.0.0", p + "transition1.1.0.1", stride=2)]
        self.stage2 = [self._module(pk, "%sstage2.%d" % (p, m), s2) for m in range(s2["NUM_MODULES"])]
        self.t2 = pk.conv(p + "transition2.2.0.0", p + "transition2.2.0.1", stride=2)
        self.stage3 = [self._module(pk, "%sstage3.%d" % (p, m), s3) for m in range(s3["NUM_MODULES"])]

    @staticmethod
    def _module(pk, q, st):
        nb = st["NUM_BRANCHES"]
        mod = dict(nb=nb, blocks=[], fuse={})
        for i in range(nb):
            mod["blocks"].append([(pk.conv("%s.branches.%d.%d.conv1" % (q, i, b), "%s.branches.%d.%d.bn1" % (q, i, b)),
                                   pk.conv("%s.branches.%d.%d.conv2" % (q, i, b), "%s.branches.%d.%d.bn2" % (q, i, b)))
                                  for b in range(st["NUM_BLOCKS"][i])])
        for i in range(nb):
            for j in range(nb):
                if j > i:
                    mod["fuse"][(i, j)] = pk.conv("%s.fuse_layers.%d.%d.0" % (q, i, j), "%s.fuse_layers.%d.%d.1" % (q, i, j))
                elif j < i:
                    mod["fuse"][(i, j)] = [pk.conv("%s.fuse_layers.%d.%d.%d.0" % (q, i, j, k),
                                                   "%s.fuse_layers.%d.%d.%d.1" % (q, i, j, k), stride=2)
                                           for k in range(i - j)]
        return mod

    @staticmethod
    def _close(P, x):
        if not isinstance(x, _PendingFuse):
            return x
        y = P.alloc(x.base.n, x.base.h, x.base.w, x.base.c, x.base.dt)
        P.fuse_up_add(x.base, x.terms, y, relu=True)
        P.release(x.base, *x.terms)
        return y

    @staticmethod
    def _emit_module(P, mod, xs, need=None, defer=None):
        nb = mod["nb"]
        xs = list(xs)
        need = set(range(nb)) if need is None else {i % nb for i in need}
        for k in range(max(len(b) for b in mod["blocks"])):
            grp, ts, folded = [], {}, []
            for i in range(nb):
                if k < len(mod["blocks"][i]):
                    if isinstance(xs[i], _PendingFuse):
                        pf = xs[i]
                        xs[i] = P.alloc(pf.base.n, pf.base.h, pf.base.w, pf.base.c, pf.base.dt)
                        ts[i] = P.conv(pf.base, mod["blocks"][i][k][0], relu=True, group=grp, fuse_in=(pf.terms, xs[i]))
                        folded.append(pf)
                        continue
                    ts[i] = P.conv(xs[i], mod["blocks"][i][k][0], relu=True, group=grp)
            P.flush_group(grp)
            for pf in folded:
                P.release(pf.base, *pf.terms)
            for i, t in ts.items():
                y = P.conv(t, mod["blocks"][i][k][1], relu=True, res1=xs[i], group=grp)
                P.release(t, xs[i])
                xs[i] = y
            P.flush_group(grp)
        xs = [HRNetW48._close(P, x) for x in xs]
        terms, ups = [], []
        for i in range(nb):
            ts = []
            for j in range(i if i in need else 0):
                chain = mod["fuse"][(i, j)]
                ts.append(dict(j=j, mids=list(chain[:-1]), last=chain[-1], cur=None))
            ts.sort(key=lambda t: (len(t["mids"]), t["j"]))
            terms.append(ts)
            ups.append([(j, mod["fuse"][(i, j)]) for j in range(i + 1, nb)] if i in need else [])
        n_up = sum(len(u) for u in ups)
        ys = [None] * nb
        n_sum = [0] * nb
        tmaps = [[] for _ in range(nb)]
        levels_left = max([1 + len(t["mids"]) for ts in terms for t in ts] + [1 if n_up else 0])
        while levels_left > 0:
            levels_left -= 1
            grp, rel = [], []
            for i in range(nb):
                ready = [t for t in terms[i] if not t["mids"]]
                for t in terms[i]:
                    if t["mids"]:
                        src = t["cur"] if t["cur"] is not None else xs[t["j"]]
                        nxt = P.conv(src, t["mids"].pop(0), relu=True, group=grp)
                        if t["cur"] is not None:
                            rel.append(t["cur"])
                        t["cur"] = nxt
                if ready:
                    t = ready[0]
                    terms[i].remove(t)
                    src = t["cur"] if t["cur"] is not None else xs[t["j"]]
                    if ys[i] is None:
                        ys[i] = P.alloc(xs[i].n, xs[i].h, xs[i].w, xs[i].c, xs[i].dt)
                    P.conv(src, t["last"], relu=(not terms[i] and not ups[i]), res1=xs[i] if n_sum[i] == 0 else ys[i], out=ys[i], group=grp)
                    n_sum[i] += 1
                    if t["cur"] is not None:
                        rel.append(t["cur"])
            if levels_left == 0 and n_up:
                cands = [(i, j, pc) for i in range(nb) for j, pc in ups[i]]
                if len(grp) + len(cands) > cabi.MAX_GROUP:
                    P.flush_group(grp)
                for i, j, pc in cands:
                    tmaps[i].append(P.conv(xs[j], pc, group=grp))
                    if len(grp) == cabi.MAX_GROUP:
                        P.flush_group(grp)
            P.flush_group(grp)
            P.release(*rel)
        assert not any(terms)
        kept = []
        for i in range(nb):
            if not tmaps[i]:
                continue
            base = xs[i] if ys[i] is None else ys[i]
            if FUSE_IN and defer is not None and defer[i] is not None and P.fuse_in_ok(base, tmaps[i], defer[i]):
                if ys[i] is None:
                    kept.append(xs[i])
                ys[i] = _PendingFuse(base, list(tmaps[i]))
                continue
            if ys[i] is None:
                ys[i] = P.alloc(xs[i].n, xs[i].h, xs[i].w, xs[i].c, xs[i].dt)
            pend = list(tmaps[i])
            while pend:
                now, pend = pend[:2], pend[2:]
                P.fuse_up_add(base, now, ys[i], relu=not pend)
                base = ys[i]
            P.release(*tmaps[i])
        P.release(*[x for x in xs if not any(x is k for k in kept)])
        return ys

    def emit(self, P, n, h, w, n_src=None, need=None):
        a, stem_args = P.stem(self.stem1, n, h, w, n_src=n_src, out_dt=P.store_dt)
        x = P.stem_conv2_layer1(a, self.conv2, self.layer1)
        grp = []
        xs = [P.conv(x, self.t1[0], relu=True, group=grp), P.conv(x, self.t1[1], relu=True, group=grp)]
        P.flush_group(grp)
        P.release(x)
        if not PRUNE_FUSE:
            need = None
        mods = list(self.stage2) + list(self.stage3)
        def first_convs(m, nb):
            nxt = mods[m + 1]["blocks"] if m + 1 < len(mods) else []
            return [nxt[i][0][0] if i < len(nxt) and nxt[i] else None for i in range(nb)]
        for m, mod in enumerate(self.stage2):
            xs = self._emit_module(P, mod, xs, defer=first_convs(m, mod["nb"]))
        xs[-1] = self._close(P, xs[-1])
        t = P.conv(xs[-1], self.t2, relu=True)
        xs = [xs[0], xs[1], t]
        for m, mod in enumerate(self.stage3, len(self.stage2)):
            last = m + 1 == len(mods)
            xs = self._emit_module(P, mod, xs, need=need if last else None, defer=None if last else first_convs(m, mod["nb"]))
        return xs, stem_args


class HRFormerB:

    def __init__(self, pk, p):
        from .arch_hrformer import STAGES
        b = p + "backbone."
        self.stem1 = pk.stem(b + "conv1", b + "bn1")
        self.conv2 = pk.conv(b + "conv2", b + "bn2", stride=2)
        self.layer1 = pk.bottlenecks(b + "layer1", 2)
        self.stages = []
        pre = [256]
        for sname, tname in (("stage2", "transition1"), ("stage3", "transition2"), ("stage4", "transition3")):
            st = STAGES[sname]
            ch = st["num_channels"]
            trans = []
            for i in range(st["num_branches"]):
                if i < len(pre):
                    trans.append(pk.conv("%s%s.%d.0" % (b, tname, i), "%s%s.%d.1" % (b, tname, i)) if ch[i] != pre[i] else None)
                else:
                    trans.append(pk.conv("%s%s.%d.0.0" % (b, tname, i), "%s%s.%d.0.1" % (b, tname, i), stride=2))
            mods = []
            for m in range(st["num_modules"]):
                multiscale = not (sname == "stage4" and m == st["num_modules"] - 1)
                mods.append(self._module(pk, "%s%s.%d" % (b, sname, m), st, multiscale))
            self.stages.append(dict(trans=trans, mods=mods, n_pre=len(pre)))
            pre = list(ch)

    @staticmethod
    def _module(pk, q, st, multiscale):
        nb, ch = st["num_branches"], st["num_channels"]
        mod = dict(nb=nb, n_out=nb if multiscale else 1, blocks=[], fuse={})
        for i in range(nb):
            blks = []
            for k in range(st["num_blocks"][i]):
                r = "%s.branches.%d.%d" % (q, i, k)
                fused = pk.attn_block_lp(r, ch[i], st["num_heads"][i]) if (pk.dtype != 0 and ch[i] in _HRT_FUSED_ATTN) else None
                fused_mlp = pk.mlp_block_lp(r, ch[i]) if (pk.dtype != 0 and ch[i] in _HRT_FUSED_MLP) else None
                blks.append(dict(c=ch[i], heads=st["num_heads"][i], ln1=pk.ln(r + ".norm1", ch[i]), ln2=pk.ln(r + ".norm2", ch[i]), attn_lp=fused, mlp_lp=fused_mlp,
                                 qkv=pk.qkv(r + ".attn.attn", ch[i], st["num_heads"][i]),
                                 out=pk.attn_out(r + ".attn.attn", ch[i], st["num_heads"][i]),
                                 fc1=pk.conv(r + ".mlp.fc1", r + ".mlp.norm1"), dw=pk.dw(r + ".mlp.dw3x3", r + ".mlp.norm2"),
                                 fc2=pk.conv(r + ".mlp.fc2", r + ".mlp.norm3")))
            mod["blocks"].append(blks)
        for i in range(mod["n_out"]):
            for j in range(nb):
                r = "%s.fuse_layers.%d.%d" % (q, i, j)
                if j > i:
                    mod["fuse"][(i, j)] = pk.conv(r + ".0", r + ".1")
                elif j < i:
                    mod["fuse"][(i, j)] = [(pk.dw("%s.%d.0" % (r, k), "%s.%d.1" % (r, k)), pk.conv("%s.%d.2" % (r, k), "%s.%d.3" % (r, k)))
                                           for k in range(i - j)]
        return mod

    @staticmethod
    def _emit_block(P, blk, x, lane=0):
        P.lane_ctx = lane
        if blk.get("attn_lp") is not None:
            x1 = P.hrt_attn(x, blk["attn_lp"], lane=lane)
            P.release(x)
        else:
            n1 = P.layernorm(x, blk["ln1"], lane=lane, out_dt=P.store_dt)
            qkv = P.conv(n1, blk["qkv"], lane=lane, out_dt=0)
            P.release(n1)
            a = P.winattn(qkv, blk["qkv"].bias, blk["c"], blk["heads"], lane=lane)
            P.release(qkv)
            x1 = P.conv(a, blk["out"], res1=x, lane=lane)
            P.release(a, x)
        if blk.get("mlp_lp") is not None:
            x2 = P.hrt_mlp(x1, blk["mlp_lp"], lane=lane)
            P.release(x1)
            return x2
        n2 = P.layernorm(x1, blk["ln2"], lane=lane, out_dt=P.store_dt)
        h1 = P.conv(n2, blk["fc1"], act=2, lane=lane)
        P.release(n2)
        h2 = P.dwconv(h1, blk["dw"], 1, act=2, lane=lane)
        P.release(h1)
        x2 = P.conv(h2, blk["fc2"], act=2, res_post=x1, lane=lane, out_dt=0)
        P.release(h2, x1)
        return x2

    @classmethod
    def _emit_module(cls, P, mod, xs, lanes):
        nb = mod["nb"]
        xs = list(xs)
        for k in range(max(len(b) for b in mod["blocks"])):
            for i in range(nb):
                if k < len(mod["blocks"][i]):
                    xs[i] = cls._emit_block(P, mod["blocks"][i][k], xs[i], lane=i if lanes else 0)
        pre, pre_y = {}, {}
        if lanes:
            for i in range(mod["n_out"]):
                for j in range(i):
                    P.lane_ctx = j
                    cur = xs[j]
                    hops = mod["fuse"][(i, j)]
                    for k, (dw, pc) in enumerate(hops):
                        d = P.dwconv(cur, dw, 2, act=0, lane=j)
                        if cur is not xs[j]:
                            P.release(cur)
                        if k < len(hops) - 1:
                            cur = P.conv(d, pc, relu=True, lane=j)
                            P.release(d)
                    pre[(i, j)] = d
                    if j == 0 and i >= 2:
                        y0 = P.alloc(xs[i].n, xs[i].h, xs[i].w, xs[i].c)
                        P.conv(d, hops[-1][1], relu=False, out=y0, lane=j)
                        P.release(d)
                        pre_y[i] = y0
        slots, waited = {}, {}
        if lanes:
            slots = P.records(range(nb))
            waited = {l: {l} for l in range(nb)}

        def need(ln, j):
            if lanes and j not in waited[ln]:
                P.wait(ln, slots[j])
                waited[ln].add(j)
        outs = []
        for i in range(mod["n_out"]):
            ln = i if lanes else 0
            P.lane_ctx = ln
            acc, y, j = None, None, 0
            while j < nb:
                if j == i:
                    assert acc is None
                    acc = xs[i]
                    j += 1
                    continue
                if j == 0 and i in pre_y:
                    need(ln, 0)
                    acc, y, j = pre_y[i], pre_y[i], 1
                    continue
                if y is None:
                    y = P.alloc(xs[i].n, xs[i].h, xs[i].w, xs[i].c)
                if j > i:
                    ts = []
                    for jj in range(j, nb):
                        need(ln, jj)
                        ts.append(P.conv(xs[jj], mod["fuse"][(i, jj)], lane=ln))
                    for k0 in range(0, len(ts), 3):
                        P.upsample_add(ts[k0:k0 + 3], acc if k0 == 0 else y, y, act=1 if k0 + 3 >= len(ts) else 0, lane=ln)
                    P.release(*ts)
                    jn = nb
                else:
                    cur = xs[j]
                    hops = mod["fuse"][(i, j)]
                    need(ln, j)
                    for k, (dw, pc) in enumerate(hops):
                        if (i, j) in pre:
                            if k < len(hops) - 1:
                                continue
# ... 216 lines not shown
        self._capture_packs = {}
        self._sine_tables = {}
        self.tower = self.reduce = self.head = None
        self.single_stack = self.single_pos = self.single_head = self.res_layer = self.single_tokens = None
        self.single_layers, self.layers, self.deconvs = [], [], []
        self.use_pos, self.pe_mode, self.return_dict = False, None, False
        self.win_block = self.cat_fc = self.upconv = self.domain_trans = None
        self.inter_stack = "global_encoder" if self.name == "interformer_pureMulti" else "multi_global_encoder"
        self.pre_norm = bool(M["NORMALIZE_BEFORE"]) and self.name == "interformer"
        self.cat_concat = self.name == "interformer" and M["MULTI_POS_EMBEDDING"] == "cat_vec" and bool(M["USE_MULTI_POS"])
        self.window_attn = self.name == "interformer" and M["ATTENTION_TYPE"] != "default"
        self.singleformer = None
        if self.name == "hrnet":
            self.tower = HRNetW48(pk, "", M["EXTRA"])
            self.reduce = pk.conv("reduce")
        elif self.name in ("transpose_h", "hrformer"):
            self.singleformer = self.name
            self._pack_single(pk, self.name, "")
        elif self.name == "interformer_pureMulti":
            self.tower = HRNetW48(pk, "", M["EXTRA"])
            self.reduce = pk.conv("reduce")
            self.use_pos = bool(M["USE_MULTI_POS"])
            if self.use_pos:
                self._pack_pos(pk, "position_embedding", M["MULTI_POS_EMBEDDING"])
            self.layers = [self._enc_layer("global_encoder.layers.%d" % l) for l in range(M["ENCODER_LAYERS"])]
            self.deconvs = [pk.deconv("deconv_layers.0", "deconv_layers.1")] * 2
            self.head = pk.head("final_layer")
        elif self.name in ("interformer", "interformer_2stage"):
            sf = M["SINGLEFORMER"]
            self.singleformer = sf
            if sf:
                self._pack_single(pk, sf, "singleformer.")
            elif not sf:
                assert self.name == "interformer", "interformer_2stage always has a first stage"
                self.tower = HRNetW48(pk, "backbone.body.", M["EXTRA"])
                self.reduce = pk.conv("backbone.body.reduce")
            self.use_pos = bool(M["USE_MULTI_POS"])
            if self.use_pos:
                self._pack_pos(pk, "multi_position_embedding", M["MULTI_POS_EMBEDDING"])
            wide = d + (M["MULTI_POS_EMBEDDING_DIM"] if self.cat_concat else 0)
            if self.window_attn:
                self.win_block = self._fp32_packer().window_block("multi_global_encoder.attn.attn", d, M["N_HEAD"])
            else:
                self.layers = [self._enc_layer("multi_global_encoder.layers.%d" % l, self.pre_norm, d=wide) for l in range(M["ENCODER_MULTI_LAYERS"])]
            if self.cat_concat:
                self.cat_fc = pk.conv("fc")
            up = M["UPSAMPLE_TYPE"]
            if up == "deconv" and self.name == "interformer_2stage":
                w4 = M["IMAGE_SIZE"][0] // 4
                n = int(math.log(w4 // (w4 >> int(math.log(w4 // M["TRANS_SIZE"][-1], 2))), 2))
                self.deconvs = [pk.deconv("deconv_layers%d.0" % (i + 1), "deconv_layers%d.1" % (i + 1)) for i in range(n)]
            elif up == "deconv":
                n = int(math.log(M["HEATMAP_SIZE"][0] // M["TRANS_SIZE"][1], 2))
                self.deconvs = [pk.deconv("upsample_layer.deconv_layers.%d.0" % i, "upsample_layer.deconv_layers.%d.1" % i)
                                for i in range(n)]
            elif up == "multiplex":
                self.deconvs = [pk.deconv("deconv_layers.0", "deconv_layers.1")] * 2
            elif up == "upconv":
                q = "upsample_layer" if self.name == "interformer" else "upsample_conv"
                self.upconv = dict(scale=M["HEATMAP_SIZE"][0] // M["TRANS_SIZE"][1], fuse=pk.conv(q + ".fuse_layers.0", q + ".fuse_layers.1"),
                                   c1=pk.conv(q + ".double_conv.0", q + ".double_conv.1"), c2=pk.conv(q + ".double_conv.3", q + ".double_conv.4"))
            else:
                raise NotImplementedError("UPSAMPLE_TYPE=%r" % up)
            self.head = pk.head("final_layer")
            if self.name == "interformer_2stage" and M["DOMAIN_TRANS"]:
                self.domain_trans = (pk.conv("domain_trans_1"), pk.conv("domain_trans_2"))
            self.return_dict = bool(M["INTER_SUPERVISION"]) and not M["SINGLEFORMER_FIX"] and bool(sf)
        else:
            raise NotImplementedError("MODEL.NAME=%r" % self.name)

    def _enc_layer(self, p, pre_norm=False, d=None):
        M = self.cfg["MODEL"]
        d, dff, heads = d or M["DIM_MODEL"], M["DIM_FEEDFORWARD"], M["N_HEAD"]
        if heads == 1 and not pre_norm and _r16(d) in (96, 80) and _r16(dff) == 192:
            return self._pk.encoder_layer(p, d, dff)
        return self._fp32_packer().encoder_layer_mh(p, d, dff, heads)

    def _fp32_packer(self):
        if self._pk32 is None:
            self._pk32 = self._pk if self._pk.dtype == 0 else Packer(self._pk.sd, self.device, "fp32")
        return self._pk32

    def capture_stacks(self):
        out = {}
        if self.single_layers:
            out[self.single_stack] = len(self.single_layers)
        if self.layers:
            out[self.inter_stack] = len(self.layers)
        return out

    def capture_map_sizes(self, H, W):
        M, out = self.cfg["MODEL"], {}
        fh = fw = None
        if self.single_layers:
            r = 4 * 2 ** self.res_layer
            fh, fw = H // r, W // r
            out[self.single_stack] = (fh, fw)
        elif self.singleformer:
            fh, fw = H // 4, W // 4
        if self.layers:
            if fh is None:
                fh, fw = H // self.tower.stride, W // self.tower.stride
            else:
                for _ in range(int(math.log(fw // M["TRANS_SIZE"][-1], 2))):
                    fh, fw = (fh + 1) // 2, (fw + 1) // 2
            out[self.inter_stack] = (fh, fw)
        return out

    def _capture_spec(self, capture, stack, layers, d=None):
        want = sorted(i for st, i in capture if st == stack)
        if not want:
            return None
        cache = self._capture_packs
        packs = {}
        for i in want:
            L = layers[i]
            if not L.get("mh"):
                if (stack, i) not in cache:
                    M = self.cfg["MODEL"]
                    cache[(stack, i)] = self._fp32_packer().encoder_layer_mh("%s.layers.%d" % (stack, i), L["d"] if d is None else d, M["DIM_FEEDFORWARD"], M["N_HEAD"])
                L = cache[(stack, i)]
            packs[i] = L
        return dict(stack=stack, layers=packs)

    def _check_capture(self, capture):
        stacks = self.capture_stacks()
        capture = frozenset((str(st), int(i)) for st, i in capture)
        for st, i in capture:
            if st not in stacks or not 0 <= i < stacks[st]:
                raise ValueError("capture (%r, %d): this model's encoder stacks are %s" % (st, i, stacks))
        return capture

    def _pack_single(self, pk, sf, p):
        M = self.cfg["MODEL"]
        d, dff = M["DIM_MODEL"], M["DIM_FEEDFORWARD"]
        if sf == "transpose_h":
            self.tower = HRNetW48(pk, p, M["EXTRA"])
            self.single_stack = p + "global_encoder"
            self.res_layer = M["HRNET_RES_LAYER"]
            self.reduce = pk.conv(p + "reduce")
            w, h = M["IMAGE_SIZE"]
            self.single_tokens = (h // 2 ** self.res_layer // 4) * (w // 2 ** self.res_layer // 4)
            self.single_pos = pk.table(p + "pos_embedding", self.single_tokens, d) if M["POS_EMBEDDING"] != "none" else None
            self.single_layers = [self._enc_layer("%sglobal_encoder.layers.%d" % (p, l)) for l in range(M["ENCODER_LAYERS"])]
            self.single_head = pk.head(p + "final_layer")
        else:
            self.tower = HRFormerB(pk, p)
            self.single_head = pk.head(p + "keypoint_head.final_layer")

    def _emit_single(self, P, S, H, W, n_src, capture=()):
        if self.singleformer == "hrformer":
            xs, stem_args = self.tower.emit(P, S, H, W, n_src=n_src)
            return xs[0], stem_args
        xs, stem_args = self.tower.emit(P, S, H, W, n_src=n_src, need={self.res_layer})
        f = P.conv(xs[self.res_layer], self.reduce, out_dt=0)
        P.release(*xs)
        tok = f.h * f.w
        assert tok == self.single_tokens, "input size does not match MODEL.IMAGE_SIZE (pos_embedding rows)"
        cap = self._capture_spec(capture, self.single_stack, self.single_layers) if capture else None
        g = P.encoder(f, self.single_layers, [i * tok for i in range(S + 1)],
                      pos=self.single_pos.data_ptr() if self.single_pos is not None else 0, pos_period=tok, pos_table=self.single_pos, capture=cap)
        if cap is None:
            P.release(f)
        return g, stem_args

    def _pack_pos(self, pk, p, mode):
        self.pe_mode = mode
        if mode == "conv":
            self.pe_stem = pk.stem(p + ".conv1", p + ".bn1")
            self.pe_conv2 = pk.conv(p + ".conv2", p + ".bn2", stride=2)
        elif mode == "res":
            self.pe_res = pk.pe_res(p)
        elif mode == "sine":
            pass
        elif mode == "cat_vec":
            w, b = pk.sd[p + ".fc.weight"], pk.sd[p + ".fc.bias"]
            self.pe_fc = dict(w=pk._dev(w.float()), b=pk._dev(b.float()), vec=int(w.shape[0]))
            if not self.cat_concat and self.pe_fc["vec"] != self.cfg["MODEL"]["DIM_MODEL"]:
                raise ValueError("MULTI_POS_EMBEDDING cat_vec as an additive embedding needs MULTI_POS_EMBEDDING_DIM == DIM_MODEL (%d vs %d)"
                                 % (self.pe_fc["vec"], self.cfg["MODEL"]["DIM_MODEL"]))
        else:
            raise NotImplementedError("MULTI_POS_EMBEDDING=%r with USE_MULTI_POS" % (mode,))

    def _sine_table(self, n, h, w, d, cs):
        key = (n, h, w, d)
        cache = self._sine_tables
        if key not in cache:
            W = n * w
            area = torch.ones(1, h, W)
            y_embed = area.cumsum(1, dtype=torch.float32)
            x_embed = area.cumsum(2, dtype=torch.float32)
            half = d // 2
            y_embed = y_embed / (y_embed[:, -1:, :] + 1e-6) * (2 * math.pi)
            x_embed = x_embed / (x_embed[:, :, -1:] + 1e-6) * (2 * math.pi)
            dim_t = torch.arange(half, dtype=torch.float32)
            dim_t = 10000 ** (2 * torch.div(dim_t, 2, rounding_mode="floor") / half)
            pos_x = x_embed[:, :, :, None] / dim_t
            pos_y = y_embed[:, :, :, None] / dim_t
            pos_x = torch.stack((pos_x[:, :, :, 0::2].sin(), pos_x[:, :, :, 1::2].cos()), dim=4).flatten(3)
            pos_y = torch.stack((pos_y[:, :, :, 0::2].sin(), pos_y[:, :, :, 1::2].cos()), dim=4).flatten(3)
            tab = torch.cat((pos_y, pos_x), dim=3).reshape(h * W, d)
            out = torch.zeros(n, h * w, cs)
            out[:, :, :d] = tab.view(n, h * w, d)
            if len(cache) > 16:
                cache.clear()
            cache[key] = out.to(self.device)
        return cache[key]

    def _fill_sine(self, patch, glen, sine_n):
        pos = patch.get("pos_sine")
        if pos is None:
            return
        n = max(sine_n, 1)
        key = (n, tuple(glen))
        if patch.get("_sine_key") == key:
            return
        tab = self._sine_table(n, pos.h, pos.w, pos.c, pos.cs)
        idx = torch.tensor([q for g in glen for q in range(g)], dtype=torch.long).to(self.device, non_blocking=True)
        assert idx.numel() == pos.n
        pos.view().view(pos.n, pos.h * pos.w, pos.cs).copy_(tab[idx])
        patch["_sine_key"] = key

    def _pos_branch(self, P, n, h, w, trans_w, n_src=None, cat=None):
        if self.pe_mode == "cat_vec":
            th = h // (w // trans_w)
            out = cat if cat is not None else P.alloc(n, th, trans_w, self.pe_fc["vec"])
            return out, P.pe_cat_vec(self.pe_fc, n, h, w, th, trans_w, out, self.cfg["MODEL"]["DIM_MODEL"] if cat is not None else 0, n_src=n_src)
        if self.pe_mode == "res":
            r = self.pe_res
            a, pe_args = P.pe_res_stem(r, n, h, w, n_src=n_src)
            b = P.maxpool(a)
            P.release(a)
            for c1, c2 in r["blocks"]:
                t = P.conv(b, c1, relu=True)
                y = P.conv(t, c2, relu=True, res1=b)
                P.release(t, b)
                b = y
            a = b
            b = P.conv(a, r["conv_end"])
            P.release(a)
        else:
            a, pe_args = P.stem(self.pe_stem, n, h, w, n_src=n_src)
            b = P.conv(a, self.pe_conv2, relu=True)
            P.release(a)
        for _ in range(int(math.log(b.w // trans_w, 2))):
            c = P.maxpool(b)
            P.release(b)
            b = c
        return b, pe_args

    def _pool_to_trans(self, P, g, out=None):
        steps = int(math.log(g.w // self.cfg["MODEL"]["TRANS_SIZE"][-1], 2))
        if out is not None and steps == 0:
            raise NotImplementedError("cat_vec with a first stage whose maps already are TRANS_SIZE")
        f = g
        for i in range(steps):
            c = P.maxpool(f, out=out if i == steps - 1 else None)
            if f is not g:
                P.release(f)
            f = c
        return f

    def _new_program(self, query=None):
        P = Program(self.device)
        P.store_dt = self.store_dt
        P.query = (query[1], dict(query[3])) if query else None
        return P

    def _build(self, S, H, W, length, flip=False, part=None, capture=(), query=None):
        M = self.cfg["MODEL"]
        P = self._new_program(query)
        patch = {}
        n_src = S
        if flip:
            S, length = 2 * S, list(length) + list(length)
        bare = self.name == "interformer_pureMulti" or not self.singleformer
        assert part is None or bare
        cat, d = None, M["DIM_MODEL"]
        if self.cat_concat:
            assert part is None
            tw = M["TRANS_SIZE"][-1]
            cat = P.alloc(S, H // (W // tw), tw, d + self.pe_fc["vec"])
        if bare and part == "tail":
            f = patch["feat"] = P.alloc(S, H // self.tower.stride, W // self.tower.stride, self.reduce.cout)
            f.t.zero_()
            single_feat = None
        elif bare:
            xs, patch["x"] = self.tower.emit(P, S, H, W, n_src=n_src, need={-1})
            if cat is not None:
                assert (xs[-1].h, xs[-1].w) == (cat.h, cat.w), "cat_vec: the backbone output is not TRANS_SIZE"
            f = P.conv(xs[-1], self.reduce, out_dt=0, out=cat)
            P.release(*xs)
            single_feat = None
            if part == "tower":
                P.finalize()
                return P, patch, f
        else:
            g, patch["x"] = self._emit_single(P, S, H, W, n_src, capture)
            single_feat = g
            if self.return_dict:
                patch["single"] = P.head(g, self.single_head)
            f = self._pool_to_trans(P, g, out=cat)
        if self.window_attn:
            e = self._emit_window_block(P, patch, f, single_feat, S, H, W, length)
            return self._emit_tail(P, patch, e, single_feat)
        pos_ptr = 0
        if self.use_pos and self.pe_mode == "sine":
            pos = patch["pos_sine"] = P.alloc(S, f.h, f.w, f.c)
            pos.t.zero_()
            pos_ptr = pos.ptr
        elif self.use_pos:
            pos, patch["pos_mask"] = self._pos_branch(P, S, H, W, M["TRANS_SIZE"][-1], n_src=n_src, cat=cat)
            assert (pos.h, pos.w, pos.cs) == (f.h, f.w, f.cs)
            pos_ptr = pos.ptr if cat is None else 0
        cap = self._capture_spec(capture, self.inter_stack, self.layers, d=f.c) if capture else None
        e = P.encoder(f, self.layers, self._token_offsets(length, f.h * f.w), pos=pos_ptr, regroupable=True, pre_norm=self.pre_norm, capture=cap)
        if cat is not None:
            t = P.conv(e, self.cat_fc, out_dt=0)
            P.release(e)
            e = t
        return self._emit_tail(P, patch, e, single_feat)

    def _emit_window_block(self, P, patch, f, single_feat, S, H, W, length):
        M, L = self.cfg["MODEL"], self.win_block
        assert sum(length) == S and f.n == S
        B, Pm, hw = len(length), max(length), f.h * f.w
        starts = [sum(length[:b]) for b in range(B)]
        pad_map = [starts[b] + q if q < length[b] else -1 for b in range(B) for q in range(Pm)]
        xp = P.rows_gather(f, pad_map)
        if f is not single_feat:
            P.release(f)
        pos_p = None
        if self.use_pos:
            pos, patch["pos_mask"] = self._pos_branch(P, S + 1, H, W, M["TRANS_SIZE"][-1], n_src=S + 1)
            assert (pos.h, pos.w, pos.cs) == (xp.h, xp.w, xp.cs)
            pos_p = P.rows_gather(pos, [m if m >= 0 else S for m in pad_map])
            P.release(pos)
        qk = P.conv(xp, L["qk"], in2=pos_p)
        v = P.conv(xp, L["v"])
        P.release(xp)
        if pos_p is not None:
            P.release(pos_p)
        att = P.alloc(B * Pm, f.h, f.w, L["hs"])
        goff = torch.zeros(B + 1, dtype=torch.int32, device=self.device)
        klen = torch.tensor([n * hw for n in length], dtype=torch.int32).to(self.device)
        P.keep += [goff, klen, L]
        a = cabi.MhAttnArgs(qk.ptr, v.ptr, att.ptr, goff.data_ptr(), 0, L["heads"], L["hp"], L["hs"], qk.cs, v.cs, att.cs, 0, 0, 0, klen.data_ptr())
        P.ops.append((cabi.OP_MH_ATTN, 0, a))
        P._register_stack(dict(descs=[], mh=[a], goff=goff, current=None), [b * Pm * hw for b in range(B + 1)])
        P.release(qk, v)
        o = P.conv(att, L["o"])
        P.release(att)
        e = P.view_scramble(o, [b * Pm + q for b in range(B) for q in range(length[b])], B, Pm, M["DIM_MODEL"])
        P.release(o)
        return e

    def _emit_tail(self, P, patch, e, single_feat):
        dtr, uc = self.domain_trans, self.upconv
        res_feat = single_feat if dtr is None else None
        if uc is not None:
            u = P.conv(e, uc["fuse"], up=uc["scale"])
            P.release(e)
            t = P.conv(u, uc["c1"], relu=True)
            P.release(u)
            e = P.conv(t, uc["c2"], relu=True, res_post=res_feat)
            P.release(t)
        for i, dc in enumerate(self.deconvs):
            last = i == len(self.deconvs) - 1
            u = P.deconv(e, dc, relu=True, res_post=res_feat if (last and res_feat is not None) else None)
            P.release(e)
            e = u
        if dtr is not None:
            t = P.conv(single_feat, dtr[0], out_dt=0)
            u = P.conv(e, dtr[1], res1=t, out_dt=0)
            P.release(e, t)
            e = u
        patch["multi"] = P.head(e, self.head)
        P.finalize()
        return P, patch

    def forward_backbone(self, x):
        assert self.name == "hrnet" and x.dim() == 4 and x.shape[1] == 3 and x.dtype == torch.float32
        S, _, H, W = x.shape
        x = x.to(self.device).contiguous()
        key = (S, H, W, "backbone")
        with torch.cuda.device(self.device):
            def build():
                P = self._new_program()
                xs, px = self.tower.emit(P, S, H, W, n_src=S, need={-1})
                f = P.conv(xs[-1], self.reduce, out_dt=0)
                P.release(*xs)
                P.finalize()
                return (P, px, f)
            P, px, f = self._program(key, build)
            px.in_ = x.data_ptr()
            P.run()
            return f.t.view(S, f.h, f.w, f.cs)[..., :f.c].permute(0, 3, 1, 2).contiguous()

    def forward_single(self, x, capture=None, queries=None):
        assert self.name in ("transpose_h", "hrformer") and x.dim() == 4 and x.shape[1] == 3 and x.dtype == torch.float32
        S, _, H, W = x.shape
        x = x.to(self.device).contiguous()
        capture = self._check_capture(capture) if capture else frozenset()
        query = self._check_queries(queries, capture)
        key = (S, H, W, "single") + (("capture", capture) if capture else ()) + (query or ())
        with torch.cuda.device(self.device):
            def build():
                P = self._new_program(query)
                g, px = self._emit_single(P, S, H, W, S, capture)
                hd = P.head(g, self.single_head)
                P.finalize()
                return (P, px, g, hd)
            P, px, g, hd = self._program(key, build)
            px.in_ = x.data_ptr()
            J = self.cfg["MODEL"]["NUM_JOINTS"]
            hm = torch.empty(S, J, g.h, g.w, dtype=torch.float32, device=self.device)
            hd.out = hm.data_ptr()
            if query:
                self._check_map_sizes(P, H, W)
                _, maps, inputs = P.set_query_capture([[g.h * g.w] * S], queries)
            elif capture:
                _, maps, inputs = P.set_capture([[g.h * g.w] * S])
            P.run(self.side_streams if P.uses_lanes else None)
            feat = g.t.view(S, g.h, g.w, g.cs)[..., :g.c].permute(0, 3, 1, 2).contiguous()
            if capture:
                return (feat, hm), self._capture_result(maps, inputs, S)
        return feat, hm

    def _check_queries(self, queries, capture):
        if queries is None:
            return None
        if not capture:
            raise ValueError("queries= needs capture=: the (stack, layer) set whose maps to query")
        mode, stacks = int(queries.mode), sorted({st for st, _ in capture})
        missing = set(stacks) - set(queries.tokens)
        if missing:
            raise ValueError("queries.tokens has no table for %s" % sorted(missing))
        up = queries.upsample
        try:
            scales = tuple((st, int(up[st] if isinstance(up, dict) else up)) for st in stacks)
        except KeyError as e:
            raise ValueError("queries.upsample has no scale for stack %s" % e)
        if mode not in (0, 1) or not all(1 <= r <= 64 for _, r in scales):
            raise ValueError("queries: mode %r (0 dependency, 1 affect), upsample %r (1 .. 64)" % (queries.mode, up))
        return ("query", mode, int(queries.capacity), scales)

    def _check_map_sizes(self, P, H, W):
        sizes = self.capture_map_sizes(H, W)
        for cap in P.captures:
            if sizes.get(cap["stack"]) != (cap["x"].h, cap["x"].w):
                raise RuntimeError("capture_map_sizes(%d, %d)[%r] = %s, but the program's stack input is %d x %d"
                                   % (H, W, cap["stack"], sizes.get(cap["stack"]), cap["x"].h, cap["x"].w))

    @staticmethod
    def _capture_result(maps, inputs, S):
        out = dict(maps)
        for st, a in inputs.items():
            out[(st, "input")] = a.view()[:S, :, :, :a.c].permute(0, 3, 1, 2).contiguous()
        return out

    @staticmethod
    def capacity(S):
        if S <= 8:
            return S
        step = 2 if S <= 32 else (4 if S <= 64 else 8)
        return -(-S // step) * step

    MAX_PROGRAMS = 48
    MAX_PROGRAM_BYTES = 32 << 30

    def forward(self, x, pos_mask, length, flip_joint_map=None, capture=None, queries=None):
        assert x.dim() == 4 and x.shape[1] == 3 and x.dtype == torch.float32
        S, _, H, W = x.shape
        assert S == sum(length), "sum(length)=%d != number of crops %d" % (sum(length), S)
        assert all(n >= 1 for n in length), "every image needs at least one person"
        sine_n = max(length)
        if capture:
            capture = self._check_capture(capture)
            assert flip_joint_map is None and not self.window_attn, "attention maps: no flip test, no window-type block"
            query = self._check_queries(queries, capture)
            with torch.cuda.device(self.device):
                return self._forward_part(x, pos_mask, list(length), None, S, H, W, sine_n, capture=capture, queries=queries, query=query)
        if queries is not None:
            self._check_queries(queries, capture)
        if self.window_attn and flip_joint_map is not None:
            with torch.cuda.device(self.device):
                x = x.to(self.device)
                pm = pos_mask.to(self.device) if pos_mask is not None else None
                a = self._forward(x, pm, list(length), None, S, H, W, sine_n)
                b = self._forward(torch.flip(x, dims=[3]), torch.flip(pm, dims=[3]) if pm is not None else None, list(length), None, S, H, W, sine_n)
                return self._flip_merge(_multi(a).contiguous(), _multi(b).contiguous(), flip_joint_map, S, H, W)
        with torch.cuda.device(self.device):
            return self._forward(x, pos_mask, list(length), flip_joint_map, S, H, W, sine_n)

    def _flip_merge(self, a, b, flip_joint_map, S, H, W):
        J = self.cfg["MODEL"]["NUM_JOINTS"]
        merged = torch.empty(S, J, H // 4, W // 4, dtype=torch.float32, device=self.device)
        cabi.check(cabi.lib().i2r_flip_merge(a.data_ptr(), b.data_ptr(), flip_joint_map.data_ptr(), merged.data_ptr(),
                                             S, J, H // 4, W // 4, torch.cuda.current_stream(self.device).cuda_stream), "i2r_flip_merge")
        return merged

    @staticmethod
    def _token_offsets(glen, tok):
        offs = [0]
        for n in glen:
            offs.append(offs[-1] + n * tok)
        return offs

    SPLIT_MIN_CROPS = 24
    SPLIT_MIN_PART = 8
    SPLIT_PARTS = 2

    def _split_bounds(self, length, H=None, W=None):
        from .dist import shard_bounds
        parts = min(self.SPLIT_PARTS, len(length))
        if parts < 2 or sum(length) < self.SPLIT_MIN_CROPS or not isinstance(self.tower, HRNetW48):
            return None
        if H is not None and (H % self.tower.stride or W % self.tower.stride):
            return None
        if self.cat_concat or self.window_attn:
            return None
        bounds = shard_bounds(list(length), parts)
        if not all(bounds[i + 1] > bounds[i] for i in range(parts)):
            return None
        if min(sum(length[bounds[i]:bounds[i + 1]]) for i in range(parts)) < self.SPLIT_MIN_PART:
            return None
        return bounds

    def _forward(self, x, pos_mask, length, flip_joint_map, S, H, W, sine_n):
        bounds = self._split_bounds(length, H, W)
        if bounds is None:
            return self._forward_part(x, pos_mask, length, flip_joint_map, S, H, W, sine_n, slot=0)
        if self.name == "interformer_pureMulti" or not self.singleformer:
            return self._forward_split(x, pos_mask, length, flip_joint_map, S, H, W, sine_n, bounds)
        parts = len(bounds) - 1
        offs = [sum(length[:b]) for b in bounds]
        x = x.to(self.device).contiguous()
        pm = pos_mask.to(self.device, torch.float32).contiguous() if pos_mask is not None else None
        progs = [None] * parts

        def run_part(i):
            y = self._forward_part(x[offs[i]:offs[i + 1]], pm[offs[i]:offs[i + 1]] if pm is not None else None,
# ... 278 lines not shown
```

intra-and-inter-human-relation-network-for-mpee_amd/pack.py:

```python
import torch


def _m16(c):
    return (c + 15) // 16 * 16


def _r16(c):
    n = (c + 15) // 16
    while not any(n % k == 0 for k in (3, 4, 5)):
        n += 1
    return 16 * n


def fold_bn(w, bn, conv_bias=None, eps=1e-5):
    w = w.double()
    cout = w.shape[0]
    b = conv_bias.double() if conv_bias is not None else torch.zeros(cout, dtype=torch.float64)
    if bn is not None:
        gamma, beta, mean, var = [t.double() for t in bn]
        scale = gamma / torch.sqrt(var + eps)
        w = w * scale.view(-1, *([1] * (w.dim() - 1)))
        b = (b - mean) * scale + beta
    return w, b


def pack_k4(w_taps, cin_pad, cout_pad):
    nt, cin, cout = w_taps.shape
    full = torch.zeros(nt, cin_pad, cout_pad, dtype=torch.float64)
    full[:, :cin, :cout] = w_taps
    return full.view(nt, cin_pad // 4, 4, cout_pad).permute(0, 1, 3, 2).contiguous().float()


PRECISIONS = {"fp32": 0, "bf16": 1, "fp16": 2}


def pack_frag(m):
    rows, cols = m.shape
    assert rows % 16 == 0 and cols % 16 == 0
    v = m.reshape(rows // 16, 16, cols // 16, 4, 4)
    return v.permute(0, 2, 3, 1, 4).contiguous().reshape(rows, cols)


def pack_frag32(m):
    rows, cols = m.shape
    assert rows % 16 == 0 and cols % 32 == 0
    v = m.reshape(rows // 16, 16, cols // 32, 4, 8)
    return v.permute(0, 2, 3, 1, 4).contiguous().reshape(rows, cols)


def pack_k8(w_taps, cin_pad, cout_pad, tdtype):
    nt, cin, cout = w_taps.shape
    g8_pad = (cin_pad // 8 + 3) // 4 * 4
    full = torch.zeros(nt, g8_pad * 8, cout_pad, dtype=torch.float64)
    full[:, :cin, :cout] = w_taps
    return full.float().to(tdtype).view(nt, g8_pad, 8, cout_pad).permute(0, 1, 3, 2).contiguous()


def winograd_weights(wf):
    G = torch.tensor([[1.0, 0.0, 0.0], [0.5, 0.5, 0.5], [0.5, -0.5, 0.5], [0.0, 0.0, 1.0]], dtype=torch.float64)
    U = torch.einsum("ia,ocab,jb->ijco", G, wf.double(), G)
    return U.reshape(16, wf.shape[1], wf.shape[0])


class PackedConv:
    __slots__ = ("w", "bias", "cin", "cin_pad", "cout", "cout_pad", "taps", "iy0", "ix0", "stride", "ksize", "dtype", "w_wino", "w_frag", "w_lp1")

    def __init__(self, w, bias, cin, cout, taps, iy0, ix0, stride, ksize, cin_pad=None, dtype=0):
        self.w, self.bias = w, bias
        self.cin, self.cin_pad = cin, (w.shape[1] * 4 if cin_pad is None else cin_pad)
        self.cout, self.cout_pad = cout, w.shape[2]
        self.taps, self.iy0, self.ix0, self.stride, self.ksize = taps, iy0, ix0, stride, ksize
        self.dtype = dtype
        self.w_wino = None
        self.w_lp1 = None
        self.w_frag = None


class Packer:
    def __init__(self, sd, device, precision="fp32"):
        self.sd = {k: v.detach().to("cpu") for k, v in sd.items()}
        self.device = device
        self.dtype = PRECISIONS[precision]

    def _pc(self, w_taps, bias, cin, cout, taps, iy0, ix0, stride, ksize):
        cin_pad, cout_pad = _r16(cin), _r16(cout)
        if self.dtype == 0:
            w = pack_k4(w_taps, cin_pad, cout_pad)
        else:
            w = pack_k8(w_taps, cin_pad, cout_pad, torch.bfloat16 if self.dtype == 1 else torch.float16)
        pc = PackedConv(self._dev(w), bias, cin, cout, taps, iy0, ix0, stride, ksize, cin_pad=cin_pad, dtype=self.dtype)
        if self.dtype != 0 and ksize == 1 and stride == 1 and w_taps.shape[0] == 1 and cin_pad >= 64 and any((cout_pad // 16) % k == 0 for k in (3, 4, 5, 6)):
            full = torch.zeros(cout_pad, (cin_pad + 31) // 32 * 32, dtype=torch.float64)
            full[:cout, :cin] = w_taps[0].t()
            pc.w_lp1 = self._dev(pack_frag32(full).float().to(torch.bfloat16 if self.dtype == 1 else torch.float16))
        return pc

    def _bn(self, key):
        if key is None:
            return None
        s = self.sd
        return (s[key + ".weight"], s[key + ".bias"], s[key + ".running_mean"], s[key + ".running_var"])

    def _dev(self, t):
        return t.contiguous().to(self.device)

    def _bias(self, b, n):
        bias = torch.zeros(n, dtype=torch.float64)
        bias[:b.shape[0]] = b
        return self._dev(bias.float())

    def conv(self, conv_key, bn_key=None, stride=1, eps=1e-5):
        w = self.sd[conv_key + ".weight"]
        cout, cin, kh, kw = w.shape
        assert kh == kw and kh in (1, 3)
        wf, bf = fold_bn(w, self._bn(bn_key), self.sd.get(conv_key + ".bias"), eps)
        taps = [(dy, dx) for dy in range(kh) for dx in range(kw)]
        w_taps = wf.permute(2, 3, 1, 0).reshape(kh * kw, cin, cout)
        cout_pad = _r16(cout)
        pad = kh // 2
        pc = self._pc(w_taps, self._bias(bf, cout_pad), cin, cout, taps, -pad, -pad, stride, kh)
        nfrag = cout_pad // 16
        if self.dtype == 0 and kh == 3 and stride == 1 and (nfrag % 3 == 0 or nfrag % 4 == 0):
            pc.w_wino = self._dev(pack_k4(winograd_weights(wf), _r16(cin), cout_pad))
        return pc

    def conv_cat(self, parts, eps=1e-5):
        mats, bias_sum, cins = [], None, []
        for conv_key, bn_key in parts:
            w = self.sd[conv_key + ".weight"]
            cout, cin, kh, kw = w.shape
            assert kh == 1 and kw == 1
            wf, bf = fold_bn(w, self._bn(bn_key), self.sd.get(conv_key + ".bias"), eps)
            mats.append(wf.reshape(cout, cin).t())
            bias_sum = bf if bias_sum is None else bias_sum + bf
            cins.append(cin)
        assert all(c % 16 == 0 for c in cins), "concatenated inputs must keep whole 16-channel steps"
        w_taps = torch.cat(mats, 0).unsqueeze(0)
        cout = w_taps.shape[2]
        pc = self._pc(w_taps, self._bias(bias_sum, _r16(cout)), sum(cins), cout, [(0, 0)], 0, 0, 1, 1)
        pc.w_frag = self._frag(w_taps)
        return pc

    def _frag(self, w_taps):
        _, cin, cout = w_taps.shape
        if self.dtype != 0 or w_taps.shape[0] != 1 or cin % 16 or cout % 16:
            return None
        return self._dev(pack_frag(w_taps[0].t().contiguous()).float())

    def bottlenecks(self, prefix, n):
        blocks = []
        for b in range(n):
            q = "%s.%d" % (prefix, b)
            blk = dict(c1=self.conv(q + ".conv1", q + ".bn1"), c2=self.conv(q + ".conv2", q + ".bn2"))
            if (q + ".downsample.0.weight") in self.sd:
                blk["c3ds"] = self.conv_cat([(q + ".downsample.0", q + ".downsample.1"), (q + ".conv3", q + ".bn3")])
            else:
                blk["c3"] = self.conv(q + ".conv3", q + ".bn3")
            for key in ("c1", "c3"):
                if key in blk:
                    w = self.sd[q + ".conv%s.weight" % key[1]]
                    wf, _ = fold_bn(w, self._bn(q + ".bn%s" % key[1]), None, 1e-5)
                    blk[key].w_frag = self._frag(wf.reshape(1, w.shape[0], w.shape[1]).permute(0, 2, 1))
            blocks.append(blk)
        return blocks

    def linear_as_conv(self, w, b):
        cout, cin = w.shape
        return self._pc(w.double().t().reshape(1, cin, cout), self._bias(b, _r16(cout)), cin, cout, [(0, 0)], 0, 0, 1, 1)

    def deconv(self, deconv_key, bn_key, eps=1e-5):
        w = self.sd[deconv_key + ".weight"]
        cin, cout, kh, kw = w.shape
        assert kh == kw and kh in self.DECONV_TAPS, "ConvTranspose2d kernel %dx%d (the reference's _get_deconv_cfg knows 2, 3, 4)" % (kh, kw)
        wf, bf = fold_bn(w.permute(1, 0, 2, 3), self._bn(bn_key), self.sd.get(deconv_key + ".bias"), eps)
        bias = self._bias(bf, _r16(cout))
        out = {}
        for py in (0, 1):
            for px in (0, 1):
                (iy0, kys), (ix0, kxs) = self.DECONV_TAPS[kh][py], self.DECONV_TAPS[kh][px]
                taps = [(dy, dx) for dy in range(len(kys)) for dx in range(len(kxs))]
                w_taps = torch.stack([wf[:, :, kys[dy], kxs[dx]].t() for dy, dx in taps], 0)
                out[(py, px)] = self._pc(w_taps, bias, cin, cout, taps, iy0, ix0, 1, max(len(kys), len(kxs)))
        return out

    DECONV_TAPS = {4: {0: (-1, (3, 1)), 1: (0, (2, 0))},
                   3: {0: (0, (1,)), 1: (0, (2, 0))},
                   2: {0: (0, (0,)), 1: (0, (1,))}}

    def stem(self, conv_key, bn_key, eps=1e-5):
        w = self.sd[conv_key + ".weight"]
        cout, cin = w.shape[:2]
        wf, bf = fold_bn(w, self._bn(bn_key), None, eps)
        return dict(w=self._dev(wf.permute(2, 3, 1, 0).reshape(9, cin, cout).float()), bias=self._dev(bf.float()),
                    cin=cin, cout=cout)

    def pe_res(self, p):
        w_pre = self.sd[p + ".conv_pre.weight"]
        assert tuple(w_pre.shape) == (3, 1, 3, 3)
        w7 = self.sd[p + ".res.0.weight"]
        assert tuple(w7.shape) == (64, 3, 7, 7)
        wf, bf = fold_bn(w7, self._bn(p + ".res.1"), None, 1e-5)
        blocks = []
        for b in range(2):
            q = "%s.res.4.%d" % (p, b)
            blocks.append((self.conv(q + ".conv1", q + ".bn1"), self.conv(q + ".conv2", q + ".bn2")))
        return dict(w_pre=self._dev(w_pre.view(3, 9).t().contiguous().float()),
                    w7=self._dev(wf.permute(2, 3, 1, 0).reshape(49 * 3, 64).float()), bias=self._dev(bf.float()), cout=64,
                    blocks=blocks, conv_end=self.conv(p + ".conv_end"))

    def head(self, key):
        w = self.sd[key + ".weight"]
        cout, cin, kh, kw = w.shape
        assert kh == kw and kh in (1, 3), "final_layer kernel %dx%d" % (kh, kw)
        if kh == 3:
            cp = 48
            assert cout <= 32
            w_taps = torch.zeros(9, cin, cp, dtype=torch.float64)
            w_taps[:, :, :cout] = w.double().permute(2, 3, 1, 0).reshape(9, cin, cout)
            taps = [(dy, dx) for dy in range(3) for dx in range(3)]
            pc = self._pc(w_taps, self._bias(self.sd[key + ".bias"], cp), cin, cp, taps, -1, -1, 1, 3)
            if self.dtype == 0:
                wf = torch.zeros(cp, cin, 3, 3, dtype=torch.float64)
                wf[:cout] = w.double()
                pc.w_wino = self._dev(pack_k4(winograd_weights(wf), _r16(cin), cp))
            eye = torch.zeros(cout, cp)
            eye[torch.arange(cout), torch.arange(cout)] = 1.0
            return dict(w=self._dev(eye), bias=self._dev(torch.zeros(cout)), cin=cp, cout=cout, conv3=pc)
        cin_pad = _r16(cin)
        wp = torch.zeros(cout, cin_pad)
        wp[:, :cin] = w.view(cout, cin)
        return dict(w=self._dev(wp), bias=self._dev(self.sd[key + ".bias"].float()), cin=cin_pad, cout=cout)

    def encoder_layer(self, p, d, dff):
        cs, fs = _r16(d), _r16(dff)
        s = self.sd

        def padm(m, r, c):
            o = torch.zeros(r, c)
            o[:m.shape[0], :m.shape[1]] = m
            return o

        def padv(v, n):
            o = torch.zeros(n)
            o[:v.shape[0]] = v
            return o

        wi, bi = s[p + ".self_attn.in_proj_weight"], s[p + ".self_attn.in_proj_bias"]
        w_in = torch.cat([padm(wi[i * d:(i + 1) * d], cs, cs) for i in range(3)], 0)
        b_in = torch.cat([padv(bi[i * d:(i + 1) * d], cs) for i in range(3)], 0)
        t = dict(
            w_in=w_in, b_in=b_in,
            w_out=padm(s[p + ".self_attn.out_proj.weight"], cs, cs), b_out=padv(s[p + ".self_attn.out_proj.bias"], cs),
            ln1_w=padv(s[p + ".norm1.weight"], cs), ln1_b=padv(s[p + ".norm1.bias"], cs),
            w1=padm(s[p + ".linear1.weight"], fs, cs), b1=padv(s[p + ".linear1.bias"], fs),
            w2=padm(s[p + ".linear2.weight"], cs, fs), b2=padv(s[p + ".linear2.bias"], cs),
            ln2_w=padv(s[p + ".norm2.weight"], cs), ln2_b=padv(s[p + ".norm2.bias"], cs))
        lp = {}
        if self.dtype != 0:
            tdt = torch.bfloat16 if self.dtype == 1 else torch.float16
            csp = 96
            assert cs <= csp and fs == 192

            def perm(m):
                rows, cols = m.shape
                v = m.view(rows, cols // 32, 2, 4, 4)
                v = v.permute(0, 1, 3, 2, 4).reshape(rows // 16, 16, cols // 32, 4, 8)
                return v.permute(0, 2, 3, 1, 4).reshape(rows, cols).to(tdt).contiguous()
            w_in_p = torch.cat([padm(wi[i * d:(i + 1) * d], csp, csp) for i in range(3)], 0)
            b_in_p = torch.cat([padv(bi[i * d:(i + 1) * d], csp) for i in range(3)], 0)
            lp = dict(w_in_lp=perm(w_in_p), w_out_lp=perm(padm(s[p + ".self_attn.out_proj.weight"], csp, csp)),
                      w1_lp=perm(padm(s[p + ".linear1.weight"], fs, csp)), w2_lp=perm(padm(s[p + ".linear2.weight"], csp, fs)),
                      vec_lp=torch.cat([b_in_p, padv(s[p + ".self_attn.out_proj.bias"], csp), padv(s[p + ".norm1.weight"], csp),
                                        padv(s[p + ".norm1.bias"], csp), padv(s[p + ".linear1.bias"], fs), padv(s[p + ".linear2.bias"], csp),
                                        padv(s[p + ".norm2.weight"], csp), padv(s[p + ".norm2.bias"], csp)]).float())
            lp = {k: self._dev(v) for k, v in lp.items()}
        for k in ("w_in", "w_out", "w1", "w2"):
            t[k] = pack_frag(t[k])
        t = {k: self._dev(v.float()) for k, v in t.items()}
        t.update(lp)
        t.update(d=d, cs=cs, dff_pad=fs, dtype=self.dtype if lp else 0)
        return t

    @staticmethod
    def mh_width(heads, hd):
        hp = _m16(hd)
        f = heads * hp // 16
        while not any(f % k == 0 for k in (3, 4, 5)):
            f += 1
        return hp, 16 * f

    def _head_padded(self, d, heads, q, k, v, o):
        hd = d // heads
        assert hd * heads == d, "nn.MultiheadAttention: embed_dim %d must be divisible by num_heads %d" % (d, heads)
        hp, hs = self.mh_width(heads, hd)
        rows = torch.tensor([hh * hp + j for hh in range(heads) for j in range(hd)])
        wqk, bqk = torch.zeros(2 * hs, d, dtype=torch.float64), torch.zeros(2 * hs, dtype=torch.float64)
        wqk[rows], bqk[rows] = q[0].double() * float(hd) ** -0.5, q[1].double() * float(hd) ** -0.5
        wqk[hs + rows], bqk[hs + rows] = k[0].double(), k[1].double()
        wv, bv = torch.zeros(hs, d, dtype=torch.float64), torch.zeros(hs, dtype=torch.float64)
        wv[rows], bv[rows] = v[0].double(), v[1].double()
        wo = torch.zeros(d, hs, dtype=torch.float64)
        wo[:, rows] = o[0].double()
        return dict(heads=heads, hp=hp, hs=hs, d=d, cs=_r16(d), qk=self.linear_as_conv(wqk, bqk), v=self.linear_as_conv(wv, bv),
                    o=self.linear_as_conv(wo, o[1]))

    def encoder_layer_mh(self, p, d, dff, heads):
# ... 126 lines not shown
```

Before: 8810 images/sec.

## Add Winograd F(2x4,3x3) conv kernel path for large 3x3 stride-1 convs

Adds a second Winograd variant that tiles 2x4 outputs per transform (24 transformed taps instead of 16), with its own LDS staging, input and output transforms, and weight packing. It is enabled by default for backbone stage classes whose launch has enough workgroups. The intent is to cut the MFMA work per output pixel relative to F(2x2,3x3). The cost is larger transformed weights, more register pressure, possible fp32 precision loss from the bigger transform, and no fused-input support, so convs with fused inputs fall back to the old path.

```diff
diff --git a/intra-and-inter-human-relation-network-for-mpee_amd/csrc/i2r_conv.h b/intra-and-inter-human-relation-network-for-mpee_amd/csrc/i2r_conv.h
--- a/intra-and-inter-human-relation-network-for-mpee_amd/csrc/i2r_conv.h
+++ b/intra-and-inter-human-relation-network-for-mpee_amd/csrc/i2r_conv.h
@@ -60,6 +60,8 @@
     asm volatile("s_nop 1" ::"v"(v));
 }
 
+constexpr int kW24Pitch = 7, kW24Strip = 127, kW24Plane = 256;
+
 constexpr int kMaxPP = 5;
 
 constexpr int kMaxGroups = 4;
diff --git a/intra-and-inter-human-relation-network-for-mpee_amd/csrc/i2r_conv.hip b/intra-and-inter-human-relation-network-for-mpee_amd/csrc/i2r_conv.hip
--- a/intra-and-inter-human-relation-network-for-mpee_amd/csrc/i2r_conv.hip
+++ b/intra-and-inter-human-relation-network-for-mpee_amd/csrc/i2r_conv.hip
@@ -310,31 +310,41 @@
     const int nt = nfrag % 3 == 0 ? 3 : (nfrag % 4 == 0 ? 4 : 0);
     I2R_CHECK_ARG(nt != 0, "i2r_conv: algo 1 needs cout_pad=%d to be a multiple of 48 or 64", d->cout_pad);
     const int mt = force_mt ? force_mt : (d->mt ? d->mt : 1);
-    I2R_CHECK_ARG(mt == 1, "i2r_conv: algo 1 takes mt 1 (got %d)", mt);
+    I2R_CHECK_ARG(mt == 1 || mt == 2, "i2r_conv: algo 1 takes mt 1 (F(2x2, 3x3)) or mt 2 (F(2x4, 3x3)) (got %d)", mt);
     I2R_CHECK_ARG(d->seq >= 0 && d->seq <= kWinoMaxSeq, "i2r_conv: algo 1 runs 1..%d fragments per workgroup (seq=%d; 0 = choose)", kWinoMaxSeq, d->seq);
-    int fw = 0;
-    if (d->tile_w) {
-        I2R_CHECK_ARG(d->tile_w == 16 || d->tile_w == 8 || d->tile_w == 4, "i2r_conv: algo 1 fragment width %d (16, 8, 4)", d->tile_w);
-        fw = d->tile_w / 2;
+    copy_desc(d, k);
+    k.n_cblk = nfrag / nt;
+    k.w_bytes = (unsigned)((long long)(mt == 2 ? 24 : 16) * d->cin * d->cout_pad * 4);
+    if (mt == 2) {
+        I2R_CHECK_ARG(!d->t1 && !d->t2 && !d->y, "i2r_conv: algo 1 mt 2 has no fused-input form (t1, t2, y)");
+        I2R_CHECK_ARG(d->seq <= 1, "i2r_conv: algo 1 mt 2 runs one fragment per workgroup (seq=%d)", d->seq);
+        I2R_CHECK_ARG(d->tile_w == 0 || d->tile_w == 4, "i2r_conv: algo 1 mt 2 strip width %d (4)", d->tile_w);
+        I2R_CHECK_ARG((long long)24 * d->cin * d->cout_pad < (1ll << 29), "i2r_conv: algo 1 mt 2 weights of < 2 GiB");
+        k.w_fwlog = 0;
+        k.tile_w = 4; k.tile_h = 16;
+        k.w_pitch = kW24Pitch; k.w_half = kW24Strip; k.plane = kW24Plane;
     } else {
-        long long best = -1;
-        for (int cand : {8, 4, 2}) {
-            const long long n = (long long)cdiv(d->conv_w, 2 * cand) * cdiv(d->conv_h, 32 / cand);
-            if (best < 0 || n < best) { best = n; fw = cand; }
-        }
-    }
-    copy_desc(d, k);
-    k.w_fwlog = fw == 8 ? 3 : (fw == 4 ? 2 : 1);
-    k.tile_w = 2 * fw; k.tile_h = 32 / fw;
+        int fw = 0;
+        if (d->tile_w) {
+            I2R_CHECK_ARG(d->tile_w == 16 || d->tile_w == 8 || d->tile_w == 4, "i2r_conv: algo 1 fragment width %d (16, 8, 4)", d->tile_w);
+            fw = d->tile_w / 2;
+        } else {
+            long long best = -1;
+            for (int cand : {8, 4, 2}) {
+                const long long n = (long long)cdiv(d->conv_w, 2 * cand) * cdiv(d->conv_h, 32 / cand);
+                if (best < 0 || n < best) { best = n; fw = cand; }
+            }
+        }
+        k.w_fwlog = fw == 8 ? 3 : (fw == 4 ? 2 : 1);
+        k.tile_w = 2 * fw; k.tile_h = 32 / fw;
+        k.w_half = fw + 1;
+        k.w_pitch = fw == 8 ? 20 : (fw == 4 ? 10 : 9);
+        k.plane = cdiv((k.tile_h + 2) * k.w_pitch, 16) * 16;
+    }
     k.tiles_x = cdiv(d->conv_w, k.tile_w); k.tiles_y = cdiv(d->conv_h, k.tile_h);
-    k.n_cblk = nfrag / nt;
     k.ph = k.tile_h + 2; k.pw = k.tile_w + 2;
-    k.w_half = fw + 1;
-    k.w_pitch = fw == 8 ? 20 : (fw == 4 ? 10 : 9);
-    k.plane = cdiv(k.ph * k.w_pitch, 16) * 16;
     k.w_rcp = (65536 + k.pw - 1) / k.pw;
     k.in_bytes = (unsigned)((long long)d->n_img * d->in_h * d->in_w * d->in_cs * 4);
-    k.w_bytes = (unsigned)((long long)16 * d->cin * d->cout_pad * 4);
     k.out_bytes = (unsigned)((long long)d->n_img * d->out_h * d->out_w * d->out_cs * 4);
     if (d->t1) k.f_bytes1 = (unsigned)((long long)d->n_img * (d->in_h >> d->t1_shift) * (d->in_w >> d->t1_shift) * d->in_cs * 4);
     if (d->t2) k.f_bytes2 = (unsigned)((long long)d->n_img * (d->in_h >> d->t2_shift) * (d->in_w >> d->t2_shift) * d->in_cs * 4);
@@ -359,6 +369,7 @@
 }
 
 static void wino_choose_seq(ConvK* g, const i2r_conv_desc* const* descs, int n, int mt) {
+    if (mt == 2) return;
     auto total = [&]() { long long t = 0; for (int i = 0; i < n; ++i) t += wino_runs(g[i], mt) * g[i].n_cblk; return t; };
     long long at_one = 0;
     for (int i = 0; i < n; ++i) at_one += ((long long)g[i].w_nfrag + mt - 1) / mt * g[i].n_cblk;
diff --git a/intra-and-inter-human-relation-network-for-mpee_amd/csrc/i2r_conv_wino.hip b/intra-and-inter-human-relation-network-for-mpee_amd/csrc/i2r_conv_wino.hip
--- a/intra-and-inter-human-relation-network-for-mpee_amd/csrc/i2r_conv_wino.hip
+++ b/intra-and-inter-human-relation-network-for-mpee_amd/csrc/i2r_conv_wino.hip
@@ -1,4 +1,5 @@
 #include "i2r_conv.h"
+#include <type_traits>
 
 namespace {
 
@@ -343,14 +344,231 @@
     }
 }
 
+template <int NT>
+__device__ __forceinline__ void conv_wino24_body(const ConvGroupK& grp) {
+    extern __shared__ __attribute__((aligned(16))) f32x4 lds[];
+    const int tid = threadIdx.x, lane = tid & 63;
+    const int wi = __builtin_amdgcn_readfirstlane(tid >> 6);
+    const int li = lane & 15, g = lane >> 4;
+
+    int bid = blockIdx.x, gi = 0;
+    if (grp.blk_map) {
+        const int v = __builtin_amdgcn_readfirstlane(grp.blk_map[bid]);
+        gi = v >> 24;
+        bid = v & 0xFFFFFF;
+    } else {
+        int start = 0;
+#pragma unroll
+        for (int i = 0; i < kMaxGroups - 1; ++i)
+            if (i + 1 < grp.n && bid >= grp.blk_end[i]) { gi = i + 1; start = grp.blk_end[i]; }
+        bid -= start;
+    }
+    const ConvK& p = grp.g[gi];
+    int wg, cb;
+    if (grp.blk_map) {
+        wg = div_m(bid, p.n_cblk, p.w_m_cblk);
+        cb = bid - wg * p.n_cblk;
+    } else {
+        const int q = bid >> 3, qq = div_m(q, p.n_cblk, p.w_m_cblk);
+        cb = q - qq * p.n_cblk;
+        wg = (bid & 7) * p.w_band + qq;
+    }
+    if (2 * wg >= p.w_nfrag) return;
+    const int n_base = cb * NT * 16;
+
+    int f_img[2], f_oy[2], f_ox[2];
+    bool f_ok[2];
+#pragma unroll
+    for (int s = 0; s < 2; ++s) {
+        int fid = 2 * wg + s;
+        f_ok[s] = fid < p.w_nfrag;
+        if (!f_ok[s]) fid = 0;
+        f_img[s] = div_m(fid, p.tiles_y * p.tiles_x, p.w_m_img);
+        const int rem = fid - f_img[s] * (p.tiles_y * p.tiles_x);
+        const int fy = div_m(rem, p.tiles_x, p.w_m_tx);
+        f_oy[s] = fy * 16;
+        f_ox[s] = (rem - fy * p.tiles_x) * 4;
+    }
+    constexpr int NIT = (2 * kWinoPatchMax * 4 + 255) / 256;
+    const __amdgpu_buffer_rsrc_t rs_in = make_rsrc(p.in, p.in_bytes), rs_w = make_rsrc(p.w, p.w_bytes);
+    unsigned goff[NIT];
+    int lslot[NIT];
+    const int cg = tid & 3;
+#pragma unroll
+    for (int k = 0; k < NIT; ++k) {
+        const int pix = (tid + k * 256) >> 2;
+        const int s = pix >= kWinoPatchMax ? (pix >= 2 * kWinoPatchMax ? 2 : 1) : 0;
+        const int pp = pix - s * kWinoPatchMax;
+        const int row = (pp * 10923) >> 16, col = pp - row * 6;
+        lslot[k] = s < 2 ? cg * kW24Plane + s * kW24Strip + row * kW24Pitch + col : -1;
+        const bool s1 = s == 1;
+        const int iy = (s1 ? f_oy[1] : f_oy[0]) - 1 + row, ix = (s1 ? f_ox[1] : f_ox[0]) - 1 + col;
+        const bool in_img = s < 2 && (s1 ? f_ok[1] : f_ok[0]) && (unsigned)iy < (unsigned)p.in_h && (unsigned)ix < (unsigned)p.in_w;
+        goff[k] = in_img ? (unsigned)((((s1 ? f_img[1] : f_img[0]) * p.in_h + iy) * p.in_w + ix) * p.in_cs + cg * 4) * 4u : kOOB;
+    }
+    f32x4 v[NIT];
+    auto stage_load = [&](int c0) {
+#pragma unroll
+        for (int k = 0; k < NIT; ++k) v[k] = buf_ld16(rs_in, goff[k], c0 * 4);
+    };
+    auto stage_store = [&](f32x4* buf) {
+#pragma unroll
+        for (int k = 0; k < NIT; ++k)
+            if (lslot[k] >= 0) buf[lslot[k]] = v[k];
+    };
+
+    const int ra = wi == 0 ? 0 : (wi == 2 ? 2 : 1);
+    const int rb = wi == 0 ? 2 : (wi == 1 ? 2 : (wi == 2 ? 1 : 3));
+    const float sg = __int_as_float(__builtin_amdgcn_readfirstlane(wi == 1 ? 0x3f800000 : 0xbf800000));
+    const int abase = g * kW24Plane + (li >> 3) * kW24Strip + 2 * (li & 7) * kW24Pitch;
+    const int oa = abase + ra * kW24Pitch, ob = abase + rb * kW24Pitch;
+    auto load_a = [&](const f32x4* buf, f32x4 (&a)[6]) {
+        f32x4 R[6];
+#pragma unroll
+        for (int c = 0; c < 6; ++c) R[c] = buf[oa + c] + sg * buf[ob + c];
+        const f32x4 e1 = R[4] - 4.f * R[2], o1 = R[3] - 4.f * R[1];
+        const f32x4 e2 = R[4] - R[2], o2 = R[3] - R[1];
+        a[0] = 4.f * R[0] - 5.f * R[2] + R[4];
+        a[1] = e1 + o1;
+        a[2] = e1 - o1;
+        a[3] = e2 + 2.f * o2;
+        a[4] = e2 - 2.f * o2;
+        a[5] = 4.f * R[1] - 5.f * R[3] + R[5];
+    };
+
+    const int cin4 = p.cin >> 2;
+    const unsigned wlane = (unsigned)(n_base + li + g * p.cout_pad) * 16u;
+    int wp = wi * 6 * cin4 * p.cout_pad * 16;
+    const int inc_j = cin4 * p.cout_pad * 16;
+    const int inc_wrap = (4 - 5 * cin4) * p.cout_pad * 16;
+    constexpr int NB = NT == 4 ? 2 : NT, NH = NT / NB;
+    f32x4 bq[2][NB];
+    constexpr int QL = NT == 4 ? 8 : 0;
+    auto fetch_b = [&](f32x4 (&b)[NB], int h) {
+#pragma unroll
+        for (int n = 0; n < NB; ++n) b[n] = buf_ld16(rs_w, wlane, wp + (h * NB + n) * 256);
+    };
+
+    f32x4 acc[6][NT];
+    const int npass = p.cin >> 4;
+    constexpr int bufsz = 4 * kW24Plane;
+    auto run_pass = [&](int pass, auto first) {
+        f32x4* cur = lds + (pass & 1) * bufsz;
+        f32x4* nxt = lds + ((pass + 1) & 1) * bufsz;
+        const bool more = pass + 1 < npass;
+        f32x4 a[6];
+        load_a(cur, a);
+#pragma unroll
+        for (int q = 0; q < 6 * NH; ++q) {
+            const int j = q / NH, h = q % NH;
+            if (q == QL) {
+                if constexpr (QL != 0) __builtin_amdgcn_sched_barrier(0);
+                if (more) stage_load((pass + 1) * 16);
+            }
+            if (q + 1 < 6 * NH) {
+                if ((q + 1) % NH == 0) wp += inc_j;
+                fetch_b(bq[(q + 1) & 1], (q + 1) % NH);
+            } else if (more) {
+                wp += inc_wrap;
+                fetch_b(bq[0], 0);
+            }
+#pragma unroll
+            for (int e = 0; e < 4; ++e)
+#pragma unroll
+                for (int n = 0; n < NB; ++n)
+                    acc[j][h * NB + n] = mfma16(a[j][e], bq[q & 1][n][e], (decltype(first)::value && e == 0) ? (f32x4){0.f, 0.f, 0.f, 0.f} : acc[j][h * NB + n]);
+        }
+        if (more) stage_store(nxt);
+        __syncthreads();
+    };
+    stage_load(0);
+    fetch_b(bq[0], 0);
+    stage_store(lds);
+    __syncthreads();
+    run_pass(0, std::true_type());
+    for (int pass = 1; pass < npass; ++pass) run_pass(pass, std::false_type());
+
+    f32x4 t[4][NT];
+#pragma unroll
+    for (int nt = 0; nt < NT; ++nt) {
+        const f32x4 s12 = acc[1][nt] + acc[2][nt], d12 = acc[1][nt] - acc[2][nt];
+        const f32x4 s34 = acc[3][nt] + acc[4][nt], d34 = acc[3][nt] - acc[4][nt];
+        t[0][nt] = acc[0][nt] + s12 + s34;
+        t[1][nt] = d12 + 2.f * d34;
+        t[2][nt] = s12 + 4.f * s34;
+        t[3][nt] = d12 + 8.f * d34 + acc[5][nt];
+    }
+    float* const Tl = reinterpret_cast<float*>(lds);
+    constexpr int TW = NT * 16;
+    constexpr int TPL = 8 * TW;
+    const bool tail = n_base + NT * 16 > p.cout || n_base + NT * 16 > p.out_cs;
+    const unsigned out_bytes = p.out_bytes;
+    const __amdgpu_buffer_rsrc_t rs_out = make_rsrc(p.out, out_bytes), rs_r1 = make_rsrc(p.res1, out_bytes), rs_r2 = make_rsrc(p.res2, out_bytes),
+                                 rs_rp = make_rsrc(p.res_post, out_bytes);
+    int lane_f;
+    asm volatile("v_mbcnt_lo_u32_b32 %0, -1, 0\n\tv_mbcnt_hi_u32_b32 %0, -1, %0" : "=v"(lane_f));
+    const int tid_f = wi * 64 + lane_f, li_f = lane_f & 15, g_f = lane_f >> 4;
+    const int q4 = tid_f & 3, px = tid_f >> 2;
+    const bool hi = (px & 4) != 0;
+    const int n0 = n_base + q4 * 4;
+    const float* const tq = Tl + ((hi ? 4 : 0) + (px & 3)) * TPL + (px >> 3) * TW + q4 * 4;
+    const float sgn = hi ? -1.f : 1.f;
+    float* const tw = Tl + (wi * 4) * TPL + ((g_f & 1) * 4) * TW + li_f;
+#pragma unroll
+    for (int s = 0; s < 2; ++s) {
+        const int oy = f_oy[s] + 2 * (px >> 3) + (hi ? 1 : 0), ox = f_ox[s] + (px & 3);
+        const bool ok = f_ok[s] && oy < p.conv_h && ox < p.conv_w;
+        const unsigned obase = ok ? (unsigned)(((f_img[s] * p.out_h + oy) * p.out_w + ox) * p.out_cs + n0) * 4u : kOOB;
+        f32x4 r[NT];
+#pragma unroll
+        for (int k = 0; k < NT; ++k) {
+            r[k] = *reinterpret_cast<const f32x4*>(p.bias + n0 + 16 * k);
+            if (p.res1) r[k] += buf_ld16(rs_r1, obase + 64u * k, 0);
+            if (p.res2) r[k] += buf_ld16(rs_r2, obase + 64u * k, 0);
+        }
+        __syncthreads();
+        if ((g_f >> 1) == s) {
+#pragma unroll
+            for (int b = 0; b < 4; ++b)
+#pragma unroll
+                for (int nt = 0; nt < NT; ++nt)
+#pragma unroll
+                    for (int e = 0; e < 4; ++e) tw[b * TPL + e * TW + nt * 16] = t[b][nt][e];
+        }
+        __syncthreads();
+#pragma unroll
+        for (int k = 0; k < NT; ++k) {
+            const float* q = tq + 16 * k;
+            const f32x4 u0 = *reinterpret_cast<const f32x4*>(q);
+            const f32x4 u1 = *reinterpret_cast<const f32x4*>(q + 4 * TPL);
+            const f32x4 u2 = *reinterpret_cast<const f32x4*>(q + 8 * TPL);
+            f32x4 y = u0 + sgn * (u1 + u2) + r[k];
+            if (p.relu) { y[0] = fmaxf(y[0], 0.f); y[1] = fmaxf(y[1], 0.f); y[2] = fmaxf(y[2], 0.f); y[3] = fmaxf(y[3], 0.f); }
+            unsigned off = obase + 64u * k;
+            if (p.res_post) y += buf_ld16(rs_rp, off, 0);
+            if (tail) {
+                const int n = n0 + 16 * k;
+                if (!(n + 4 <= p.cout || n + 4 <= p.out_cs)) off = kOOB;
+#pragma unroll
+                for (int e = 0; e < 4; ++e)
+                    if (n + e >= p.cout) y[e] = 0.f;
+            }
+            __builtin_amdgcn_raw_buffer_store_b128(__builtin_bit_cast(u32x4, y), rs_out, off, 0, 0);
+        }
+    }
+}
+
 __device__ __forceinline__ ConvKArg wino_args() {
     static_assert(offsetof(ConvGroupK, g) == 0, "the members lead the kernel argument");
     return (ConvKArg)__builtin_amdgcn_kernarg_segment_ptr();
 }
 
 template <int MT, int NT>
-__global__ __launch_bounds__(256, (MT == 1 ? (NT == 3 ? 4 : 3) : 2)) void conv_wino_f32(const ConvGroupK grp) {
-    conv_wino_body<MT, NT, false>(grp, wino_args());
+__global__ __launch_bounds__(256, (MT == 1 && NT == 3 ? 4 : 3)) void conv_wino_f32(const ConvGroupK grp) {
+    if constexpr (MT == 2)
+        conv_wino24_body<NT>(grp);
+    else
+        conv_wino_body<MT, NT, false>(grp, wino_args());
 }
 
 template <int MT, int NT>
@@ -364,10 +582,17 @@
     conv_fn fn = nullptr;
     if (mt == 1 && nt == 3) fn = fin ? conv_wino_fin_f32<1, 3> : conv_wino_f32<1, 3>;
     if (mt == 1 && nt == 4) fn = fin ? conv_wino_fin_f32<1, 4> : conv_wino_f32<1, 4>;
+    if (mt == 2 && nt == 3 && !fin) fn = conv_wino_f32<2, 3>;
+    if (mt == 2 && nt == 4 && !fin) fn = conv_wino_f32<2, 4>;
     return reinterpret_cast<void*>(fn);
 }
 
 size_t i2r_conv_wino_lds(int nt, int mt, int plane) {
+    if (mt == 2) {
+        const size_t stage = (size_t)2 * 4 * plane * 16;
+        const size_t xchg = (size_t)4 * 4 * 8 * nt * 16 * 4;
+        return stage > xchg ? stage : xchg;
+    }
     const size_t stage = (size_t)2 * mt * 4 * plane * 16;
     const size_t xchg = (size_t)4 * 2 * mt * 16 * nt * 16 * 4;
     return stage > xchg ? stage : xchg;
diff --git a/intra-and-inter-human-relation-network-for-mpee_amd/engine.py b/intra-and-inter-human-relation-network-for-mpee_amd/engine.py
--- a/intra-and-inter-human-relation-network-for-mpee_amd/engine.py
+++ b/intra-and-inter-human-relation-network-for-mpee_amd/engine.py
@@ -6,7 +6,7 @@
 
 from . import cabi
 from .pack import (PRECISIONS, PackedConv, Packer, _m16, _r16, fold_bn, pack_frag, pack_frag32, pack_k4, pack_k8,
-                   winograd_weights)
+                   winograd24_weights, winograd_weights)
 
 
 def wino_fragment(conv_h, conv_w):
@@ -27,6 +27,8 @@
 FUSE_IN = True
 PRUNE_FUSE = True
 WINOGRAD = True
+WINO_F24 = True
+WINO_F24_MIN_WG = 768
 WINO_SEQ = True
 PROFILER_ATTACHED = bool(os.environ.get("ROCP_TOOL_LIBRARIES") or os.environ.get("ROCPROFILER_LIBRARY_CTOR") or os.environ.get("HSA_TOOLS_LIB")
                          or any(t in os.environ.get("LD_PRELOAD", "") for t in ("rocprof", "roctracer", "rocprofiler")))
@@ -198,7 +200,7 @@
         return out, a
 
     def conv(self, x, pc, relu=False, res1=None, res2=None, res_post=None, in2=None, up=1, out=None, out_step=1,
-             out_off=(0, 0), out_hw=None, lane=0, group=None, act=None, out_dt=None, fuse_in=None):
+             out_off=(0, 0), out_hw=None, lane=0, group=None, act=None, out_dt=None, fuse_in=None, wino24=False):
         assert x.cs >= pc.cin_pad and x.c == pc.cin, "conv input channels %d/%d vs weight %d" % (x.c, x.cs, pc.cin)
         assert x.dt in (0, pc.dtype), "16-bit stored input needs the matching 16-bit conv (input %d, conv %d)" % (x.dt, pc.dtype)
         if (LP1X1 and pc.w_lp1 is not None and fuse_in is None and group is None and in2 is None and up == 1 and out_step == 1 and tuple(out_off) == (0, 0)
@@ -259,6 +261,12 @@
             d.tile_h, d.tile_w, d.mt, d.wn, d.ck = fh, fw, mt, 1, 0
             d.seq = 0 if WINO_SEQ else 1
             n_frag = x.n * -(-conv_h // fh) * -(-conv_w // fw)
+            if wino24:
+                if fuse_in is not None or pc.w_wino24 is None:
+                    raise ValueError("wino24 needs weights packed with wino24=True and no fuse_in")
+                mt = 2
+                d.w, d.tile_h, d.tile_w, d.mt = pc.w_wino24.data_ptr(), 16, 4, mt
+                n_frag = x.n * -(-conv_h // 16) * -(-conv_w // 4)
             geo = ("wino", -(-n_frag // mt) * (nfrag // nt))
             key = ("wino", nt, mt)
         else:
@@ -346,7 +354,7 @@
         words = c0 // 2 if a.dt else c0
         return Act(a.t[words:], a.n, a.h, a.w, c, a.cs, a.dt)
 
-    def stem_conv2_layer1(self, a, conv2, blocks):
+    def stem_conv2_layer1(self, a, conv2, blocks, wino24=False):
         first = blocks[0]
         assert "c3ds" in first, "layer1.0 carries the downsample"
         cx, cm = conv2.cout, first["c2"].cout
@@ -355,7 +363,7 @@
         self.conv(a, conv2, relu=True, out=x)
         self.release(a)
         t1 = self.conv(x, first["c1"], relu=True)
-        self.conv(t1, first["c2"], relu=True, out=t2)
+        self.conv(t1, first["c2"], relu=True, out=t2, wino24=wino24)
         def pair_ok(pa, pb):
             return (pa.w_frag is not None and pa.cin in (64, 128) and pa.cout % 32 == 0 and pa.cout == pa.cout_pad
                     and (pb is None or (pb.w_frag is not None and pb.cout == 64 and pb.cin == pa.cout)))
@@ -365,7 +373,7 @@
             y, t1 = self.conv1x1_pair(cat, first["c3ds"], None, blocks[1]["c1"] if len(blocks) > 1 else None)
             self.release(cat)
             for i, blk in enumerate(blocks[1:], 1):
-                t2 = self.conv(t1, blk["c2"], relu=True)
+                t2 = self.conv(t1, blk["c2"], relu=True, wino24=wino24)
                 self.release(t1)
                 yn, t1 = self.conv1x1_pair(t2, blk["c3"], y, blocks[i + 1]["c1"] if i + 1 < len(blocks) else None)
                 self.release(t2, y)
@@ -376,7 +384,7 @@
         x = y
         for blk in blocks[1:]:
             t1 = self.conv(x, blk["c1"], relu=True)
-            t2 = self.conv(t1, blk["c2"], relu=True)
+            t2 = self.conv(t1, blk["c2"], relu=True, wino24=wino24)
             y = self.conv(t2, blk["c3"], relu=True, res1=x)
             self.release(t1, t2, x)
             x = y
@@ -947,8 +955,8 @@
         self.stride = 4 * 2 ** (s3["NUM_BRANCHES"] - 1)
         self.stem1 = pk.stem(p + "conv1", p + "bn1")
         self.conv2 = pk.conv(p + "conv2", p + "bn2", stride=2)
-        self.layer1 = pk.bottlenecks(p + "layer1", 4)
-        self.t1 = [pk.conv(p + "transition1.0.0", p + "transition1.0.1"),
+        self.layer1 = pk.bottlenecks(p + "layer1", 4, wino24=True)
+        self.t1 = [pk.conv(p + "transition1.0.0", p + "transition1.0.1", wino24=True),
                    pk.conv(p + "transition1.1.0.0", p + "transition1.1.0.1", stride=2)]
         self.stage2 = [self._module(pk, "%sstage2.%d" % (p, m), s2) for m in range(s2["NUM_MODULES"])]
         self.t2 = pk.conv(p + "transition2.2.0.0", p + "transition2.2.0.1", stride=2)
@@ -959,8 +967,8 @@
         nb = st["NUM_BRANCHES"]
         mod = dict(nb=nb, blocks=[], fuse={})
         for i in range(nb):
-            mod["blocks"].append([(pk.conv("%s.branches.%d.%d.conv1" % (q, i, b), "%s.branches.%d.%d.bn1" % (q, i, b)),
-                                   pk.conv("%s.branches.%d.%d.conv2" % (q, i, b), "%s.branches.%d.%d.bn2" % (q, i, b)))
+            mod["blocks"].append([(pk.conv("%s.branches.%d.%d.conv1" % (q, i, b), "%s.branches.%d.%d.bn1" % (q, i, b), wino24=True),
+                                   pk.conv("%s.branches.%d.%d.conv2" % (q, i, b), "%s.branches.%d.%d.bn2" % (q, i, b), wino24=True))
                                   for b in range(st["NUM_BLOCKS"][i])])
         for i in range(nb):
             for j in range(nb):
@@ -982,12 +990,13 @@
         return y
 
     @staticmethod
-    def _emit_module(P, mod, xs, need=None, defer=None):
+    def _emit_module(P, mod, xs, need=None, defer=None, wino24=False):
         nb = mod["nb"]
         xs = list(xs)
         need = set(range(nb)) if need is None else {i % nb for i in need}
         for k in range(max(len(b) for b in mod["blocks"])):
             grp, ts, folded = [], {}, []
+            w24 = wino24 and not any(isinstance(xs[i], _PendingFuse) for i in range(nb) if k < len(mod["blocks"][i]))
             for i in range(nb):
                 if k < len(mod["blocks"][i]):
                     if isinstance(xs[i], _PendingFuse):
@@ -996,12 +1005,12 @@
                         ts[i] = P.conv(pf.base, mod["blocks"][i][k][0], relu=True, group=grp, fuse_in=(pf.terms, xs[i]))
                         folded.append(pf)
                         continue
-                    ts[i] = P.conv(xs[i], mod["blocks"][i][k][0], relu=True, group=grp)
+                    ts[i] = P.conv(xs[i], mod["blocks"][i][k][0], relu=True, group=grp, wino24=w24)
             P.flush_group(grp)
             for pf in folded:
                 P.release(pf.base, *pf.terms)
             for i, t in ts.items():
-                y = P.conv(t, mod["blocks"][i][k][1], relu=True, res1=xs[i], group=grp)
+                y = P.conv(t, mod["blocks"][i][k][1], relu=True, res1=xs[i], group=grp, wino24=wino24)
                 P.release(t, xs[i])
                 xs[i] = y
             P.flush_group(grp)
@@ -1074,11 +1083,23 @@
         P.release(*[x for x in xs if not any(x is k for k in kept)])
         return ys
 
-    def emit(self, P, n, h, w, n_src=None, need=None):
+    def wino24_classes(self, n, h, w):
+        half = lambda v: (v - 1) // 2 + 1
+        maps = [(half(half(h)), half(half(w)))]
+        maps += [(half(maps[0][0]), half(maps[0][1])), (half(half(maps[0][0])), half(half(maps[0][1])))]
+
+        def workgroups(pcs):
+            return sum(-(-(n * -(-hh // 16) * -(-ww // 4)) // 2) * (pc.cout_pad // 16 // (3 if pc.cout_pad // 16 % 3 == 0 else 4)) for pc, (hh, ww) in zip(pcs, maps))
+        launches = {"layer1": [self.layer1[0]["c2"]], "transition1": [self.t1[0]], "stage2": [b[0][0] for b in self.stage2[0]["blocks"]],
+                    "stage3": [b[0][0] for b in self.stage3[0]["blocks"]]}
+        return tuple(c for c, pcs in launches.items() if all(pc.w_wino24 is not None for pc in pcs) and workgroups(pcs) >= WINO_F24_MIN_WG)
+
+    def emit(self, P, n, h, w, n_src=None, need=None, wino24=False):
         a, stem_args = P.stem(self.stem1, n, h, w, n_src=n_src, out_dt=P.store_dt)
-        x = P.stem_conv2_layer1(a, self.conv2, self.layer1)
+        on = lambda cls: wino24 is True or (bool(wino24) and cls in wino24)
+        x = P.stem_conv2_layer1(a, self.conv2, self.layer1, wino24=on("layer1"))
         grp = []
-        xs = [P.conv(x, self.t1[0], relu=True, group=grp), P.conv(x, self.t1[1], relu=True, group=grp)]
+        xs = [P.conv(x, self.t1[0], relu=True, group=grp, wino24=on("transition1")), P.conv(x, self.t1[1], relu=True, group=grp)]
         P.flush_group(grp)
         P.release(x)
         if not PRUNE_FUSE:
@@ -1088,13 +1109,13 @@
             nxt = mods[m + 1]["blocks"] if m + 1 < len(mods) else []
             return [nxt[i][0][0] if i < len(nxt) and nxt[i] else None for i in range(nb)]
         for m, mod in enumerate(self.stage2):
-            xs = self._emit_module(P, mod, xs, defer=first_convs(m, mod["nb"]))
+            xs = self._emit_module(P, mod, xs, defer=first_convs(m, mod["nb"]), wino24=on("stage2"))
         xs[-1] = self._close(P, xs[-1])
         t = P.conv(xs[-1], self.t2, relu=True)
         xs = [xs[0], xs[1], t]
         for m, mod in enumerate(self.stage3, len(self.stage2)):
             last = m + 1 == len(mods)
-            xs = self._emit_module(P, mod, xs, need=need if last else None, defer=None if last else first_convs(m, mod["nb"]))
+            xs = self._emit_module(P, mod, xs, need=need if last else None, defer=None if last else first_convs(m, mod["nb"]), wino24=on("stage3"))
         return xs, stem_args
 
 
@@ -1617,7 +1638,7 @@
         if self.singleformer == "hrformer":
             xs, stem_args = self.tower.emit(P, S, H, W, n_src=n_src)
             return xs[0], stem_args
-        xs, stem_args = self.tower.emit(P, S, H, W, n_src=n_src, need={self.res_layer})
+        xs, stem_args = self.tower.emit(P, S, H, W, n_src=n_src, need={self.res_layer}, wino24=WINO_F24 and self.tower.wino24_classes(S, H, W))
         f = P.conv(xs[self.res_layer], self.reduce, out_dt=0)
         P.release(*xs)
         tok = f.h * f.w
@@ -1751,7 +1772,7 @@
             f.t.zero_()
             single_feat = None
         elif bare:
-            xs, patch["x"] = self.tower.emit(P, S, H, W, n_src=n_src, need={-1})
+            xs, patch["x"] = self.tower.emit(P, S, H, W, n_src=n_src, need={-1}, wino24=WINO_F24 and self.tower.wino24_classes(S, H, W))
             if cat is not None:
                 assert (xs[-1].h, xs[-1].w) == (cat.h, cat.w), "cat_vec: the backbone output is not TRANS_SIZE"
             f = P.conv(xs[-1], self.reduce, out_dt=0, out=cat)
@@ -1852,7 +1873,7 @@
         with torch.cuda.device(self.device):
             def build():
                 P = self._new_program()
-                xs, px = self.tower.emit(P, S, H, W, n_src=S, need={-1})
+                xs, px = self.tower.emit(P, S, H, W, n_src=S, need={-1}, wino24=WINO_F24 and self.tower.wino24_classes(S, H, W))
                 f = P.conv(xs[-1], self.reduce, out_dt=0)
                 P.release(*xs)
                 P.finalize()
diff --git a/intra-and-inter-human-relation-network-for-mpee_amd/pack.py b/intra-and-inter-human-relation-network-for-mpee_amd/pack.py
--- a/intra-and-inter-human-relation-network-for-mpee_amd/pack.py
+++ b/intra-and-inter-human-relation-network-for-mpee_amd/pack.py
@@ -62,8 +62,18 @@
     return U.reshape(16, wf.shape[1], wf.shape[0])
 
 
+WINO_G4 = [[0.25, 0.0, 0.0], [-1 / 6, -1 / 6, -1 / 6], [-1 / 6, 1 / 6, -1 / 6], [1 / 24, 1 / 12, 1 / 6], [1 / 24, -1 / 12, 1 / 6], [0.0, 0.0, 1.0]]
+WINO_G2 = [[1.0, 0.0, 0.0], [0.5, 0.5, 0.5], [0.5, -0.5, 0.5], [0.0, 0.0, 1.0]]
+
+
+def winograd24_weights(wf):
+    Gy, Gx = torch.tensor(WINO_G2, dtype=torch.float64), torch.tensor(WINO_G4, dtype=torch.float64)
+    U = torch.einsum("ia,ocab,jb->ijco", Gy, wf.double(), Gx)
+    return U.reshape(24, wf.shape[1], wf.shape[0])
+
+
 class PackedConv:
-    __slots__ = ("w", "bias", "cin", "cin_pad", "cout", "cout_pad", "taps", "iy0", "ix0", "stride", "ksize", "dtype", "w_wino", "w_frag", "w_lp1")
+    __slots__ = ("w", "bias", "cin", "cin_pad", "cout", "cout_pad", "taps", "iy0", "ix0", "stride", "ksize", "dtype", "w_wino", "w_wino24", "w_frag", "w_lp1")
 
     def __init__(self, w, bias, cin, cout, taps, iy0, ix0, stride, ksize, cin_pad=None, dtype=0):
         self.w, self.bias = w, bias
@@ -72,6 +82,7 @@
         self.taps, self.iy0, self.ix0, self.stride, self.ksize = taps, iy0, ix0, stride, ksize
         self.dtype = dtype
         self.w_wino = None
+        self.w_wino24 = None
         self.w_lp1 = None
         self.w_frag = None
 
@@ -109,7 +120,7 @@
         bias[:b.shape[0]] = b
         return self._dev(bias.float())
 
-    def conv(self, conv_key, bn_key=None, stride=1, eps=1e-5):
+    def conv(self, conv_key, bn_key=None, stride=1, eps=1e-5, wino24=False):
         w = self.sd[conv_key + ".weight"]
         cout, cin, kh, kw = w.shape
         assert kh == kw and kh in (1, 3)
@@ -122,6 +133,8 @@
         nfrag = cout_pad // 16
         if self.dtype == 0 and kh == 3 and stride == 1 and (nfrag % 3 == 0 or nfrag % 4 == 0):
             pc.w_wino = self._dev(pack_k4(winograd_weights(wf), _r16(cin), cout_pad))
+            if wino24:
+                pc.w_wino24 = self._dev(pack_k4(winograd24_weights(wf), _r16(cin), cout_pad))
         return pc
 
     def conv_cat(self, parts, eps=1e-5):
@@ -147,11 +160,11 @@
             return None
         return self._dev(pack_frag(w_taps[0].t().contiguous()).float())
 
-    def bottlenecks(self, prefix, n):
+    def bottlenecks(self, prefix, n, wino24=False):
         blocks = []
         for b in range(n):
             q = "%s.%d" % (prefix, b)
-            blk = dict(c1=self.conv(q + ".conv1", q + ".bn1"), c2=self.conv(q + ".conv2", q + ".bn2"))
+            blk = dict(c1=self.conv(q + ".conv1", q + ".bn1"), c2=self.conv(q + ".conv2", q + ".bn2", wino24=wino24))
             if (q + ".downsample.0.weight") in self.sd:
                 blk["c3ds"] = self.conv_cat([(q + ".downsample.0", q + ".downsample.1"), (q + ".conv3", q + ".bn3")])
             else:
```

Result: no change. 8813 images/sec, median of 3 (+0.0%).
